# genetics-statistics/GEMMA

Measured on AMD Instinct MI355X. Metric: SNPs/s (-lmm 1 Wald) at n=20k on 1/2/4/8 MI355X; U^T x HBM GB/s vs roofline, higher is better.
Workload: dtype f64 (U^T x as int8-digit MFMA products with exact int32 accumulation; every column of U scaled by its exact maximum and rounded to 6 base-256 digits = 2^-48 of that maximum -- fp64 keeps 2^-53 per entry; value_strict / strict_leg (7g6m: U^T x at or below the fp64 GEMM's own error) and fp64_gemm_path

## Files before the change

gemma_amd/csrc/abi_lmm_multi.inc.h:

```cpp

static int multi_make_weights(hipStream_t s) {
  g_ctx.multi_G = 0;
  const size_t T = g_ctx.multi_T, c = g_ctx.cfg.n_cvt;
  const Ctx::PhenoSlot &p0 = g_ctx.slots[0];
  if (!p0.proto.have_grid || !table_v2_enabled() || p0.grid_geom.nbx != 2) return GEMMA_HIP_OK;
  const int G = std::min(MULTI_GMAX, MULTI_NBA * 16 / p0.grid_geom.nq - (int)c);
  if (G < 2 || T < 2) return GEMMA_HIP_OK;
  const GridGeom gg = p0.grid_geom;
  const size_t r_elems = (size_t)gg.nc * (size_t)(gg.nbx + MULTI_NBA) * 256;
  const size_t groups = (T + G - 1) / G;
  if (g_ctx.multi_R.reserve(groups * r_elems * 8))
    return fail(GEMMA_HIP_ENOMEM, "lmm_multi_setup: weights of the shared table (%zu bytes)", groups * r_elems * 8);
  AssocArgs k = p0.proto;
  k.eval = g_ctx.eval;
  k.UtWt = g_ctx.UtWt.as<double>();
  for (size_t grp = 0; grp < groups; ++grp) {
    MultiWeights mw;
    mw.G = (int)std::min((size_t)G, T - grp * G);
    for (int g = 0; g < MULTI_GMAX; ++g) mw.Uty[g] = g_ctx.slots[std::min(T - 1, grp * G + g)].Uty;
    hipLaunchKernelGGL(grid_weights_multi_kernel, dim3((unsigned)((r_elems + 255) / 256)), dim3(256), 0, s, k, gg, (int)c, mw,
                       g_ctx.multi_R.as<double>() + grp * r_elems);
    HIPCHK(hipGetLastError());
  }
  g_ctx.multi_G = G;
  return GEMMA_HIP_OK;
}

static int multi_setup_slots(size_t T, const double *l_mle_null, const double *logl_mle_H0, const double *UtW_d,
                             const double *UtY_d, hipStream_t s) {
  const size_t n = g_ctx.cfg.n;
  if (g_ctx.multi_Yt.reserve(T * n * 8)) return fail(GEMMA_HIP_ENOMEM, "lmm_multi_setup: U^T Y (%zu bytes)", T * n * 8);
  {
    dim3 grid((unsigned)((T + 31) / 32), (unsigned)((n + 31) / 32));
    hipLaunchKernelGGL(transpose_kernel, grid, dim3(32, 8), 0, s, UtY_d, (long)n, (long)T, (long)T, g_ctx.multi_Yt.as<double>(),
                       (long)n);
    HIPCHK(hipGetLastError());
  }
  g_ctx.slots.clear();
  g_ctx.slots.resize(T);
  g_ctx.multi_T = T;
  for (size_t t = 0; t < T; ++t) {
    Ctx::PhenoSlot &p = g_ctx.slots[t];
    p.proto = t == 0 ? g_ctx.single.proto : g_ctx.slots[0].proto;
    if (p.carry.reserve(4 * 8)) return fail(GEMMA_HIP_ENOMEM, "lmm_multi_setup: carry");
    HIPCHK(hipMemset(p.carry.p, 0, 4 * 8));
    p.carry_flip = 0;
    p.proto.l_mle_null = l_mle_null ? l_mle_null[t] : 0.0;
    p.proto.logl_mle_H0 = logl_mle_H0 ? logl_mle_H0[t] : 0.0;
    p.Uty = g_ctx.multi_Yt.as<double>() + t * n;
    const int rc = t == 0 ? make_utwt(p, UtW_d, s) : make_grid(p, s);
    if (rc == GEMMA_HIP_ENOMEM) {
      const Ctx::PhenoSlot &p0 = g_ctx.slots[0];
      const size_t per = p0.grid_R.cap + p0.grid_F.cap + p0.cheb_R.cap + p0.cheb_F.cap;
      return fail(GEMMA_HIP_ENOMEM, "lmm_multi_setup: the tables of phenotype %zu of %zu do not fit (%zu bytes per phenotype)", t + 1, T,
                  per);
    }
    if (rc) return rc;
  }
  return multi_make_weights(s);
}

static int multi_check(const gemma_lmm_cfg *cfg, size_t T, const double *l_mle_null, const double *logl_mle_H0) {
  if (!cfg) return fail(GEMMA_HIP_EINVAL, "lmm_multi_setup: null cfg");
  if (T == 0 || T > (size_t)GEMMA_LMM_MULTI_MAX)
    return fail(GEMMA_HIP_EINVAL, "lmm_multi_setup: T=%zu phenotypes (1..%d)", T, GEMMA_LMM_MULTI_MAX);
  if (cfg->a_mode != 1 && (!l_mle_null || !logl_mle_H0))
    return fail(GEMMA_HIP_EINVAL, "lmm_multi_setup: a_mode %d needs l_mle_null and logl_mle_H0 of every phenotype", cfg->a_mode);
  return GEMMA_HIP_OK;
}
static int multi_setup(const char *who, SetupSrc src, const gemma_lmm_cfg *cfg, size_t T, const double *l_mle_null,
                       const double *logl_mle_H0, const double *U, const double *eval, const double *UtW, const double *UtY,
                       hipStream_t s) {
  const double *UtW_d, *UtY_d;
  int rc = lmm_bind(who, src, cfg, U, eval, UtW, UtY, T, &UtW_d, &UtY_d);
  if (rc) return rc;
  if ((rc = multi_setup_slots(T, l_mle_null, logl_mle_H0, UtW_d, UtY_d, s))) {
    multi_release();
    return rc;
  }
  if (src != SetupSrc::Device) HIPCHK(hipDeviceSynchronize());
  g_ctx.lmm_active = true;
  return GEMMA_HIP_OK;
}

extern "C" int gemma_hip_lmm_multi_setup_d(const gemma_lmm_cfg *cfg, size_t T, const double *l_mle_null,
                                           const double *logl_mle_H0, const double *U_d, const double *eval_d,
                                           const double *UtW_d, const double *UtY_d, void *stream) {
  NEED_INIT();
  if (!U_d || !eval_d || !UtW_d || !UtY_d) return fail(GEMMA_HIP_EINVAL, "lmm_multi_setup: null pointer");
  if (int rc = multi_check(cfg, T, l_mle_null, logl_mle_H0)) return rc;
  return multi_setup("lmm_multi_setup", SetupSrc::Device, cfg, T, l_mle_null, logl_mle_H0, U_d, eval_d, UtW_d, UtY_d, S(stream));
}

extern "C" int gemma_hip_lmm_multi_setup(const gemma_lmm_cfg *cfg, size_t T, const double *l_mle_null, const double *logl_mle_H0,
                                         const double *U, const double *eval, const double *UtW, const double *UtY) {
  NEED_INIT();
  if (!U || !eval || !UtW || !UtY) return fail(GEMMA_HIP_EINVAL, "lmm_multi_setup: null pointer");
  if (int rc = multi_check(cfg, T, l_mle_null, logl_mle_H0)) return rc;
  return multi_setup("lmm_multi_setup", SetupSrc::Host, cfg, T, l_mle_null, logl_mle_H0, U, eval, UtW, UtY, nullptr);
}

extern "C" int gemma_hip_lmm_multi_setup_kept(const gemma_lmm_cfg *cfg, size_t T, const double *l_mle_null,
                                              const double *logl_mle_H0, const double *UtW, const double *UtY) {
  NEED_INIT();
  if (!g_ctx.kept_n) return fail(GEMMA_HIP_ESTATE, "lmm_multi_setup_kept: no kept U");
  if (!UtW || !UtY) return fail(GEMMA_HIP_EINVAL, "lmm_multi_setup_kept: null pointer");
  if (int rc = multi_check(cfg, T, l_mle_null, logl_mle_H0)) return rc;
  if (cfg->n != g_ctx.kept_n)
    return fail(GEMMA_HIP_EINVAL, "lmm_multi_setup_kept: cfg.n=%zu, kept U is %zu", cfg->n, g_ctx.kept_n);
  return multi_setup("lmm_multi_setup_kept", SetupSrc::Kept, cfg, T, l_mle_null, logl_mle_H0, nullptr, nullptr, UtW, UtY, nullptr);
}

static int launch_table_multi(size_t grp, int Gn, const double *UtX, size_t l, size_t ld, hipStream_t s) {
  const Ctx::PhenoSlot &p0 = g_ctx.slots[0];
  const GridGeom &gg = p0.grid_geom;
  constexpr int NB16M = (2 + MULTI_NBA) * 16;
  const size_t nb16 = (size_t)p0.proto.grid_ld;
  const int ksplit = table_ksplit(gg.nc);
  if (g_ctx.table_P.reserve((size_t)ksplit * l * NB16M * 8) || g_ctx.multi_T_buf.reserve((size_t)Gn * l * nb16 * 8))
    return fail(GEMMA_HIP_ENOMEM, "lmm_multi_batch: shared table partial sums (%zu bytes)", (size_t)ksplit * l * NB16M * 8);
  const size_t r_elems = (size_t)gg.nc * (size_t)(gg.nbx + MULTI_NBA) * 256;
  TableV2 a;
  a.UtX = UtX; a.ld = (long)ld; a.l = (long)l; a.n = (int)g_ctx.cfg.n; a.nc = gg.nc; a.ksplit = ksplit;
  a.Rp = g_ctx.multi_R.as<double>() + grp * r_elems;
  a.P = g_ctx.table_P.as<double>(); a.cap = (long)l;
  a.tg = TableGather();
  const size_t rows_per_block = (size_t)MULTI_RG * 16 * 4;
  const dim3 grid((unsigned)((l + rows_per_block - 1) / rows_per_block), (unsigned)ksplit);
  if (g_ctx.knobs.table_pf) hipLaunchKernelGGL((table_v2_kernel<2, MULTI_NBA, MULTI_RG, false, true>), grid, dim3(256), 0, s, a);
  else hipLaunchKernelGGL((table_v2_kernel<2, MULTI_NBA, MULTI_RG, false, false>), grid, dim3(256), 0, s, a);
  HIPCHK(hipGetLastError());
  TableMulti m;
  m.P = a.P; m.ksplit = ksplit; m.cap = (long)l; m.l = (long)l; m.nb16m = NB16M; m.nb16 = (int)nb16;
  m.y0 = p0.proto.grid_xa0 + (int)g_ctx.cfg.n_cvt * gg.nq; m.nq = gg.nq;
  m.T = g_ctx.multi_T_buf.as<double>(); m.tstride = (long)(l * nb16);
  hipLaunchKernelGGL(table_multi_reduce_kernel, dim3((unsigned)((l * nb16 + 255) / 256), (unsigned)Gn), dim3(256), 0, s, m);
  HIPCHK(hipGetLastError());
  return GEMMA_HIP_OK;
}

extern "C" int gemma_hip_lmm_multi_batch_d(int kind, const void *geno, size_t l, size_t ld, gemma_sumstat *out_d, void *stream) {
  NEED_INIT();
  if (!g_ctx.lmm_active || !g_ctx.multi_T) return fail(GEMMA_HIP_ESTATE, "lmm_multi_batch before lmm_multi_setup");
  if (l == 0) return GEMMA_HIP_OK;
  int rc = block_geom("lmm_multi_batch", kind, g_ctx.cfg.n, true, geno, l, ld, out_d);
  if (rc) return rc;
  hipStream_t s = S(stream);
  double *UtX;
  size_t ldx;
  if ((rc = compute_utx(kind, geno, l, ld, -1, &UtX, &ldx, s))) return rc;
  const size_t T = g_ctx.multi_T;
  bool shared = g_ctx.knobs.multi_table && g_ctx.multi_G >= 2 && table_v2_enabled() &&
                assoc_takes_tables(g_ctx.slots[0].proto, UtX, ldx);
  const size_t G = shared ? (size_t)g_ctx.multi_G : 1;
  const size_t tstride = l * (size_t)g_ctx.slots[0].proto.grid_ld;
  for (size_t t0 = 0; t0 < T; t0 += G) {
    const size_t Gn = std::min(G, T - t0);
    if (shared) {
      ProfScope ps(GEMMA_STAGE_ASSOC, s);
      rc = launch_table_multi(t0 / G, (int)Gn, UtX, l, ldx, s);
      if (rc && rc != GEMMA_HIP_ENOMEM) return rc;
      if (rc) shared = false;
    }
    for (size_t g = 0; g < Gn; ++g) {
      rc = launch_assoc(g_ctx.slots[t0 + g], UtX, l, ldx, out_d + (t0 + g) * l, s,
                        shared ? g_ctx.multi_T_buf.as<double>() + g * tstride : nullptr);
      if (rc) return rc;
    }
  }
  return GEMMA_HIP_OK;
}

extern "C" int gemma_hip_lmm_multi_batch(int kind, const void *geno, size_t l, size_t ld, gemma_sumstat *out) {
  NEED_INIT();
  if (!g_ctx.lmm_active || !g_ctx.multi_T) return fail(GEMMA_HIP_ESTATE, "lmm_multi_batch before lmm_multi_setup");
  if (l == 0) return GEMMA_HIP_OK;
  return host_batch("lmm_multi_batch", kind, geno, l, ld, g_ctx.stage_out, out, g_ctx.multi_T * l * sizeof(gemma_sumstat),
                    [&](const void *in_d, void *out_d) {
                      return gemma_hip_lmm_multi_batch_d(kind, in_d, l, ld, static_cast<gemma_sumstat *>(out_d), nullptr);
                    });
}
```

gemma_amd/csrc/abi_lmm_stage.inc.h:

```cpp

static void multi_release() {
  for (auto &p : g_ctx.slots) p.release();
  g_ctx.slots.clear();
  g_ctx.multi_Yt.release(); g_ctx.multi_R.release(); g_ctx.multi_T_buf.release();
  g_ctx.multi_T = 0;
  g_ctx.multi_G = 0;
}
static void score_release() {
  g_ctx.score_R.release(); g_ctx.score_Pyy.release(); g_ctx.score_Yt.release(); g_ctx.score_lam.release(); g_ctx.score_bad.release();
  g_ctx.score_fthr.release(); g_ctx.score_cells.release(); g_ctx.score_hits.release(); g_ctx.score_cnt.release(); g_ctx.score_best.release();
  g_ctx.score_fthr_p = -1.0;
  g_ctx.score_T = 0;
  g_ctx.refine_Yt.release(); g_ctx.refine_logl.release(); g_ctx.refine_out.release();
  g_ctx.refine_ready = false;
  g_ctx.last_UtX = nullptr;
}
static void lmm_release() {
  g_ctx.own_U.release(); g_ctx.own_eval.release(); g_ctx.own_Uty.release(); g_ctx.own_UtW.release();
  g_ctx.UtWt.release(); g_ctx.idx_map.release(); g_ctx.X.release(); g_ctx.UtX.release();
  g_ctx.stage_in.release(); g_ctx.stage_out.release(); g_ctx.scratch.release();
  g_ctx.single.release();
  g_ctx.grid_T.release();
  g_ctx.table_P.release();
  g_ctx.cheb_T.release(); g_ctx.cheb_slots.release();
  g_ctx.cheb_list.release(); g_ctx.cheb_count.release(); g_ctx.cheb_D.release(); g_ctx.cheb_Ck.release();
  g_ctx.cheb_Gk.release(); g_ctx.cheb_Lk.release(); g_ctx.cheb_iv.release(); g_ctx.cheb_dends.release(); g_ctx.cheb_res.release();
  g_ctx.i8_Bt.release(); g_ctx.i8_q.release(); g_ctx.i8_qinv.release(); g_ctx.i8_cmax.release(); g_ctx.i8_A.release(); g_ctx.i8_C.release();
  raster_release();
  g_ctx.i8_mean.release(); g_ctx.i8_meta.release(); g_ctx.i8_rowsur.release(); g_ctx.i8_colsum.release(); g_ctx.i8_surlist.release();
  g_ctx.i8_ready = g_ctx.i8_colsum_ready = false;
  g_ctx.gxe_env.release(); g_ctx.gxe_UtWt.release(); g_ctx.gxe_Z.release(); g_ctx.gxe_UtZ.release(); g_ctx.gxe_flip.release();
  g_ctx.gxe_ready = false;
  g_ctx.mv_Yt.release(); g_ctx.mv_out.release(); g_ctx.mv_scratch.release();
  g_ctx.mv_ready = g_ctx.mv_gxe = false;
  multi_release();
  score_release();
  g_ctx.U = g_ctx.eval = nullptr;
  g_ctx.U_even_of = nullptr;
  g_ctx.U_even.release();
  g_ctx.lmm_active = false;
}
#define NEED_SINGLE(who)                                                                                                 \
  do {                                                                                                                    \
    if (g_ctx.multi_T)                                                                                                    \
      return fail(GEMMA_HIP_ESTATE, who ": the setup holds %zu phenotypes (gemma_hip_lmm_multi_batch)", g_ctx.multi_T);   \
    if (g_ctx.score_T)                                                                                                    \
      return fail(GEMMA_HIP_ESTATE, who ": the setup is a score panel of %zu phenotypes (gemma_hip_lmm_score_panel_batch)", \
                  g_ctx.score_T);                                                                                         \
  } while (0)

static void fill_lam_grid(AssocArgs &a, double l_min, double l_max, size_t n_region) {
  const double lambda_interval = log(l_max / l_min) / (double)n_region;
  for (size_t i = 0; i <= n_region; ++i) a.lam_grid[i] = l_min * exp(lambda_interval * (double)i);
}
static double lnbeta_half(double df) { return lgamma(df / 2.0) + lgamma(0.5) - lgamma(df / 2.0 + 0.5); }
static void null_derive(const NullOut &h, double trace_G, size_t n, size_t n_cvt, double *out8) {
  out8[0] = h.l_mle; out8[1] = h.logl_mle; out8[2] = h.l_remle; out8[3] = h.logl_remle;
  double arg = -1.0 / h.dev2_remle, d1 = arg;
  if (arg < 0.001) d1 = fabs(arg);
  const double se = (d1 < 0.0) ? NAN : sqrt(d1);
  out8[4] = trace_G * h.l_remle / (trace_G * h.l_remle + 1.0);
  out8[5] = trace_G / ((trace_G * h.l_remle + 1.0) * (trace_G * h.l_remle + 1.0)) * se;
  out8[7] = h.Pyy_remle / (double)(n - n_cvt);
  out8[6] = out8[7] * h.l_remle;
}

static int lmm_common_setup(const gemma_lmm_cfg *cfg) {
  if (!cfg) return fail(GEMMA_HIP_EINVAL, "lmm_setup: null cfg");
  if (cfg->n == 0 || cfg->n_cvt == 0) return fail(GEMMA_HIP_EINVAL, "lmm_setup: n=%zu n_cvt=%zu", cfg->n, cfg->n_cvt);
  if (cfg->n_cvt > (size_t)GEN_CMAX_WIDE)
    return fail(GEMMA_HIP_EINVAL, "lmm_setup: n_cvt=%zu not supported by this build (1..%d)", cfg->n_cvt, GEN_CMAX_WIDE);
  if (!(cfg->a_mode == 1 || cfg->a_mode == 2 || cfg->a_mode == 3 || cfg->a_mode == 4 || cfg->a_mode == 9))
    return fail(GEMMA_HIP_EINVAL, "lmm_setup: a_mode %d", cfg->a_mode);
  if (!(cfg->l_max > cfg->l_min) || cfg->n_region == 0 || cfg->n_region > (size_t)ASSOC_MAX_REGION)
    return fail(GEMMA_HIP_EINVAL, "lmm_setup: l_min/l_max/n_region");
  if (cfg->n <= cfg->n_cvt + 1) return fail(GEMMA_HIP_EINVAL, "lmm_setup: n <= n_cvt + 1");
  if (cfg->n > 0x7fffffffUL) return fail(GEMMA_HIP_EINVAL, "lmm_setup: n too large");
  g_ctx.cfg = *cfg;
  if (g_ctx.multi_T) multi_release();
  if (g_ctx.score_T) score_release();
  {
    size_t mf = 0, mt = 0;
    if (eigh_pool_idle_bytes_x() > 0 && hipMemGetInfo(&mf, &mt) == hipSuccess && eigh_pool_idle_bytes_x() > mt / 4) (void)eigh_release_x();
  }
  g_ctx.knobs.load();
  Ctx::PhenoSlot &p = g_ctx.single;
  AssocArgs &a = p.proto;
  memset(&a, 0, sizeof a);
  a.n = (int)cfg->n;
  a.a_mode = cfg->a_mode;
  a.n_region = (int)cfg->n_region;
  a.plink_nan_rule = cfg->plink_nan_rule;
  a.l_min = cfg->l_min;
  a.l_max = cfg->l_max;
  a.l_mle_null = cfg->l_mle_null;
  a.logl_mle_H0 = cfg->logl_mle_H0;
  a.lnbeta_half_df = lnbeta_half((double)cfg->n - (double)cfg->n_cvt - 1.0);
  fill_lam_grid(a, cfg->l_min, cfg->l_max, cfg->n_region);
  if (p.carry.reserve(4 * 8)) return fail(GEMMA_HIP_ENOMEM, "lmm_setup: carry");
  HIPCHK(hipMemset(p.carry.p, 0, 4 * 8));
  p.carry_flip = 0;
  g_ctx.have_map = false;
  g_ctx.ni_total = 0;
  g_ctx.i8_ready = false;
  g_ctx.i8_colsum_ready = false;
  g_ctx.gxe_ready = false;
  g_ctx.mv_ready = false;
  return GEMMA_HIP_OK;
}

static double *kept_U() { return g_ctx.kept_UE.as<double>(); }
static double *kept_eval() { return g_ctx.kept_UE.as<double>() + g_ctx.kept_n * g_ctx.kept_n; }

enum class SetupSrc { Device, Host, Kept };

static int lmm_bind(const char *who, SetupSrc src, const gemma_lmm_cfg *cfg, const double *U, const double *eval, const double *UtW,
                    const double *UtY, size_t T, const double **UtW_d, const double **UtY_d) {
  const int rc = lmm_common_setup(cfg);
  if (rc) return rc;
  g_ctx.lmm_active = false;
  g_ctx.U_even_of = nullptr;
  if (src == SetupSrc::Device) {
    g_ctx.U = U;
    g_ctx.eval = eval;
    *UtW_d = UtW;
    *UtY_d = UtY;
    return GEMMA_HIP_OK;
  }
  const size_t n = cfg->n, c = cfg->n_cvt;
  const bool kept = src == SetupSrc::Kept;
  if ((!kept && (g_ctx.own_U.reserve(n * n * 8) || g_ctx.own_eval.reserve(n * 8))) || g_ctx.own_Uty.reserve(n * T * 8) ||
      g_ctx.own_UtW.reserve(n * c * 8))
    return fail(GEMMA_HIP_ENOMEM, "%s: cannot allocate U and U^T Y (%zu bytes)", who, (kept ? 0 : n * n * 8) + n * T * 8);
  if (!kept) {
    HIPCHK(hipMemcpy(g_ctx.own_U.p, U, n * n * 8, hipMemcpyHostToDevice));
    HIPCHK(hipMemcpy(g_ctx.own_eval.p, eval, n * 8, hipMemcpyHostToDevice));
  }
  HIPCHK(hipMemcpy(g_ctx.own_Uty.p, UtY, n * T * 8, hipMemcpyHostToDevice));
  HIPCHK(hipMemcpy(g_ctx.own_UtW.p, UtW, n * c * 8, hipMemcpyHostToDevice));
  g_ctx.U = kept ? kept_U() : g_ctx.own_U.as<double>();
  g_ctx.eval = kept ? kept_eval() : g_ctx.own_eval.as<double>();
  *UtW_d = g_ctx.own_UtW.as<double>();
  *UtY_d = g_ctx.own_Uty.as<double>();
  return GEMMA_HIP_OK;
}

static bool grid_blocks(size_t c, int nq, int *nbx, int *nba) {
  *nbx = (nq + 15) / 16;
  *nba = ((int)(c + 1) * nq + 15) / 16;
  return c >= 1 && c <= 4 && nq == 23;
}
static int make_cheb(Ctx::PhenoSlot &p, hipStream_t s) {
  AssocArgs &a = p.proto;
  a.have_cheb = 0;
  a.cheb_T = nullptr; a.cheb_F = nullptr; a.cheb_slots = nullptr; a.cheb_res = nullptr;
  if (!g_ctx.knobs.assoc_cheb) return GEMMA_HIP_OK;
  const size_t n = g_ctx.cfg.n, c = g_ctx.cfg.n_cvt;
  const int nreg = (int)g_ctx.cfg.n_region;
  const double width = log(g_ctx.cfg.l_max / g_ctx.cfg.l_min) / (double)nreg;
  if (c < 1 || c > 4 || width > 2.31 || nreg > 62) return GEMMA_HIP_OK;
  int j0 = 0;
  if (!g_ctx.knobs.cheb_lowlambda)
    while (j0 < nreg && a.lam_grid[j0] < CHEB_MIN_LAMBDA * (1.0 - 1e-9)) ++j0;
  const int nint = nreg - j0;
  p.cheb_qmask = 0;
  if (nint <= 0) return GEMMA_HIP_OK;
  GridGeom gg;
  gg.nq = CHEB_N;
  gg.nbx = (CHEB_N + 15) / 16;
  gg.nba = ((int)(c + 1) * CHEB_N + 15) / 16;
  gg.nc = (int)((n + 15) / 16);
  if (!(gg.nbx == 2 && (gg.nba == 3 || gg.nba == 5 || gg.nba == 6 || gg.nba == 8))) return GEMMA_HIP_OK;
  const size_t nb = (size_t)(gg.nbx + gg.nba);
  const size_t r_elems = (size_t)gg.nc * nb * 256;
  const size_t npairs = (c + 1) * (c + 2) / 2;
  const size_t fld = (npairs + 3) * CHEB_N;
  if (p.cheb_R.reserve((size_t)nint * r_elems * 8) || p.cheb_F.reserve((size_t)nint * fld * 8) ||
      g_ctx.cheb_D.reserve(CHEB_N * CHEB_N * 8) || g_ctx.cheb_Ck.reserve(n * CHEB_N * 8) ||
      g_ctx.cheb_Gk.reserve(2 * n * CHEB_N * 8) || g_ctx.cheb_Lk.reserve(n * CHEB_N * 8) ||
      g_ctx.cheb_iv.reserve(2 * ASSOC_MAX_REGION * 8))
    return fail(GEMMA_HIP_ENOMEM, "lmm_setup: Chebyshev tables (%zu bytes)", (size_t)nint * r_elems * 8);
  std::vector<double> D((size_t)CHEB_N * CHEB_N);
  for (int k = 0; k < CHEB_N; ++k)
    for (int m = 0; m < CHEB_N; ++m)
      D[(size_t)k * CHEB_N + m] = cos(M_PI * k * (m + 0.5) / CHEB_N) * (k == 0 ? 1.0 : 2.0) / CHEB_N;
  HIPCHK(hipMemcpyAsync(g_ctx.cheb_D.p, D.data(), D.size() * 8, hipMemcpyHostToDevice, s));
  HIPCHK(hipStreamSynchronize(s));
  AssocArgs k = a;
  k.eval = g_ctx.eval;
  k.Uty = p.Uty;
  k.UtWt = g_ctx.UtWt.as<double>();
  for (int q = 0; q < nint; ++q) {
    const ChebInterval iv = cheb_interval(a.lam_grid[j0 + q], a.lam_grid[j0 + q + 1], CHEB_MARGIN);
    p.cheb_mid[q] = iv.mid;
    p.cheb_inv_half[q] = 1.0 / iv.half;
    ChebNodes nd;
    for (int m = 0; m < CHEB_N; ++m) nd.lam[m] = exp(cheb_node(iv, m));
    const int qform = a.lam_grid[j0 + q] < CHEB_MIN_LAMBDA * (1.0 - 1e-9) ? 1 : 0;
    if (qform) p.cheb_qmask |= 1ull << q;
    double *G2k = g_ctx.cheb_Gk.as<double>() + n * CHEB_N;
    hipLaunchKernelGGL(cheb_coeff_kernel, dim3((unsigned)((n + 127) / 128)), dim3(128), 0, s, g_ctx.eval, (int)n, nd,
                       g_ctx.cheb_D.as<double>(), qform, g_ctx.cheb_Ck.as<double>(), g_ctx.cheb_Gk.as<double>(),
                       g_ctx.cheb_Lk.as<double>(), G2k);
    HIPCHK(hipGetLastError());
    hipLaunchKernelGGL(cheb_weights_kernel, dim3((unsigned)((r_elems + 255) / 256)), dim3(256), 0, s, k, gg, (int)c,
                       g_ctx.cheb_Ck.as<double>(), p.cheb_R.as<double>() + (size_t)q * r_elems);
    HIPCHK(hipGetLastError());
    hipLaunchKernelGGL(cheb_fixed_kernel, dim3((unsigned)(npairs + 3)), dim3(256), 0, s, k, (int)c,
                       g_ctx.cheb_Ck.as<double>(), g_ctx.cheb_Gk.as<double>(), g_ctx.cheb_Lk.as<double>(), G2k,
                       p.cheb_F.as<double>() + (size_t)q * fld);
    HIPCHK(hipGetLastError());
  }
  {
    std::vector<double> ivs(2 * (size_t)nint);
    for (int q = 0; q < nint; ++q) { ivs[2 * q] = p.cheb_mid[q]; ivs[2 * q + 1] = p.cheb_inv_half[q]; }
    HIPCHK(hipMemcpyAsync(g_ctx.cheb_iv.p, ivs.data(), ivs.size() * 8, hipMemcpyHostToDevice, s));
    HIPCHK(hipStreamSynchronize(s));
  }
  p.cheb_geom = gg;
  a.cheb_iv = g_ctx.cheb_iv.as<double>();
  a.cheb_logdet_off = (int)((npairs + 1) * CHEB_N);
  a.cheb_F = p.cheb_F.as<double>();
  a.cheb_ld = (int)(nb * 16);
  a.cheb_fld = (int)fld;
  a.cheb_xa0 = gg.nbx * 16;
  a.cheb_j0 = j0;
  a.cheb_nint = nint;
  a.cheb_qmask = p.cheb_qmask;
  a.cheb_final = g_ctx.knobs.assoc_final_series;
  a.have_cheb = 1;
  return GEMMA_HIP_OK;
}

static int make_grid(Ctx::PhenoSlot &p, hipStream_t s) {
  AssocArgs &a = p.proto;
  a.have_grid = 0;
  a.grid_T = nullptr;
  a.grid_F = nullptr;
  if (!g_ctx.knobs.assoc_grid) return GEMMA_HIP_OK;
  const size_t n = g_ctx.cfg.n, c = g_ctx.cfg.n_cvt;
  GridGeom gg;
  gg.nq = 1 + 2 * ((int)g_ctx.cfg.n_region + 1);
  if (!grid_blocks(c, gg.nq, &gg.nbx, &gg.nba)) return GEMMA_HIP_OK;
  gg.nc = (int)((n + 15) / 16);
  const size_t nb = (size_t)(gg.nbx + gg.nba);
  const size_t r_elems = (size_t)gg.nc * nb * 256;
  if (p.grid_R.reserve(r_elems * 8) || p.grid_F.reserve((size_t)gg.nq * GRID_FIX_LD * 8))
    return fail(GEMMA_HIP_ENOMEM, "lmm_setup: fixed-lambda table");
  AssocArgs k = a;
  k.eval = g_ctx.eval;
  k.Uty = p.Uty;
  k.UtWt = g_ctx.UtWt.as<double>();
  hipLaunchKernelGGL(grid_weights_kernel, dim3((unsigned)((r_elems + 255) / 256)), dim3(256), 0, s, k, gg, (int)c,
                     p.grid_R.as<double>());
  HIPCHK(hipGetLastError());
  hipLaunchKernelGGL(grid_fixed_kernel, dim3((unsigned)gg.nq), dim3(256), 0, s, k, (int)c, p.grid_F.as<double>());
  HIPCHK(hipGetLastError());
  p.grid_geom = gg;
  a.grid_F = p.grid_F.as<double>();
  a.grid_ld = (int)(nb * 16);
  a.grid_nq = gg.nq;
  a.grid_xa0 = gg.nbx * 16;
  a.have_grid = 1;
  return make_cheb(p, s);
}

static bool table_v2_enabled() { return g_ctx.knobs.table_v2 != 0; }
static int table_ksplit(int nc) { return std::max(1, std::min(16, nc / 32)); }
template <int NBX, int NBA, int RG>
static int launch_table_v2_t(const GridGeom &gg, const double *UtX, size_t l, size_t ld, const double *R, double *T,
                             const TableGather *tg, int nint, hipStream_t s) {
  constexpr int NB16 = (NBX + NBA) * 16;
  const size_t rows_per_block = (size_t)RG * 16 * 4;
  const size_t bx = (l + rows_per_block - 1) / rows_per_block;
  const int ksplit = table_ksplit(gg.nc);
  const size_t planes = tg ? (size_t)nint : 1;
  if (g_ctx.table_P.reserve(planes * (size_t)ksplit * l * NB16 * 8))
    return fail(GEMMA_HIP_ENOMEM, "lmm_assoc: table partial sums (%zu bytes)", planes * (size_t)ksplit * l * NB16 * 8);
  TableV2 a;
  a.UtX = UtX; a.ld = (long)ld; a.l = (long)l; a.n = (int)g_ctx.cfg.n; a.nc = gg.nc; a.ksplit = ksplit; a.Rp = R;
  a.P = g_ctx.table_P.as<double>(); a.cap = (long)l;
  if (tg) a.tg = *tg; else a.tg = TableGather();
  const long total = (long)l * NB16;
  const bool pf = g_ctx.knobs.table_pf != 0;
  if (tg) {
    if (pf) hipLaunchKernelGGL((table_v2_kernel<NBX, NBA, RG, true, true>), dim3((unsigned)bx, (unsigned)ksplit, (unsigned)nint), dim3(256), 0, s, a);
    else hipLaunchKernelGGL((table_v2_kernel<NBX, NBA, RG, true, false>), dim3((unsigned)bx, (unsigned)ksplit, (unsigned)nint), dim3(256), 0, s, a);
    HIPCHK(hipGetLastError());
    hipLaunchKernelGGL(table_reduce_kernel<true>, dim3((unsigned)((total + 255) / 256), (unsigned)nint), dim3(256), 0, s,
                       a.P, ksplit, a.cap, NB16, (long)l, tg->count, T);
  } else {
    if (pf) hipLaunchKernelGGL((table_v2_kernel<NBX, NBA, RG, false, true>), dim3((unsigned)bx, (unsigned)ksplit), dim3(256), 0, s, a);
    else hipLaunchKernelGGL((table_v2_kernel<NBX, NBA, RG, false, false>), dim3((unsigned)bx, (unsigned)ksplit), dim3(256), 0, s, a);
    HIPCHK(hipGetLastError());
    hipLaunchKernelGGL(table_reduce_kernel<false>, dim3((unsigned)((total + 255) / 256)), dim3(256), 0, s, a.P, ksplit,
                       a.cap, NB16, (long)l, (const int *)nullptr, T);
  }
  HIPCHK(hipGetLastError());
  return GEMMA_HIP_OK;
}
static int launch_table_v2(const GridGeom &gg, const double *UtX, size_t l, size_t ld, const double *R, double *T,
                           const TableGather *tg, int nint, hipStream_t s) {
  switch (gg.nba) {
  case 3: return launch_table_v2_t<2, 3, 4>(gg, UtX, l, ld, R, T, tg, nint, s);
  case 5: return launch_table_v2_t<2, 5, 2>(gg, UtX, l, ld, R, T, tg, nint, s);
  case 6: return launch_table_v2_t<2, 6, 2>(gg, UtX, l, ld, R, T, tg, nint, s);
  case 8: return launch_table_v2_t<2, 8, 2>(gg, UtX, l, ld, R, T, tg, nint, s);
  default: return fail(GEMMA_HIP_ERUNTIME, "lmm_assoc: no table kernel for %d column blocks", gg.nba);
  }
}

static int launch_grid_table(Ctx::PhenoSlot &p, const double *UtX, size_t l, size_t ld, hipStream_t s) {
  const GridGeom &gg = p.grid_geom;
  const size_t nb = (size_t)(gg.nbx + gg.nba);
  if (g_ctx.grid_T.reserve(l * nb * 16 * 8)) return fail(GEMMA_HIP_ENOMEM, "lmm_assoc: fixed-lambda table");
  const unsigned grid = (unsigned)((l + 15) / 16);
  const double *R = p.grid_R.as<double>();
  double *T = g_ctx.grid_T.as<double>();
  const int n = (int)g_ctx.cfg.n;
  if (table_v2_enabled()) return launch_table_v2(gg, UtX, l, ld, R, T, nullptr, 0, s);
  switch (gg.nba) {
  case 3: hipLaunchKernelGGL((grid_table_kernel<2, 3, false>), dim3(grid), dim3(256), 0, s, UtX, (long)ld, (long)l, n, gg.nc, R, T, TableGather()); break;
  case 5: hipLaunchKernelGGL((grid_table_kernel<2, 5, false>), dim3(grid), dim3(256), 0, s, UtX, (long)ld, (long)l, n, gg.nc, R, T, TableGather()); break;
  case 6: hipLaunchKernelGGL((grid_table_kernel<2, 6, false>), dim3(grid), dim3(256), 0, s, UtX, (long)ld, (long)l, n, gg.nc, R, T, TableGather()); break;
  case 8: hipLaunchKernelGGL((grid_table_kernel<2, 8, false>), dim3(grid), dim3(256), 0, s, UtX, (long)ld, (long)l, n, gg.nc, R, T, TableGather()); break;
  default: return fail(GEMMA_HIP_ERUNTIME, "lmm_assoc: no fixed-lambda table kernel for %d column blocks", gg.nba);
  }
  HIPCHK(hipGetLastError());
  return GEMMA_HIP_OK;
}

static int launch_cheb_tables(Ctx::PhenoSlot &p, AssocArgs &a, const double *UtX, size_t l, size_t ld, hipStream_t s) {
  const GridGeom &gg = p.cheb_geom;
  const size_t nb = (size_t)(gg.nbx + gg.nba), nint = (size_t)a.cheb_nint;
  if (g_ctx.cheb_T.reserve(nint * l * nb * 16 * 8) || g_ctx.cheb_slots.reserve(l * nint * sizeof(int)) ||
      g_ctx.cheb_list.reserve(nint * l * sizeof(int)) || g_ctx.cheb_count.reserve(ASSOC_MAX_REGION * sizeof(int)) ||
      g_ctx.cheb_dends.reserve(2 * nint * l * sizeof(double2)) || g_ctx.cheb_res.reserve(2 * nint * l * sizeof(ChebResult)))
    return fail(GEMMA_HIP_ENOMEM, "lmm_assoc: Chebyshev tables of the batch (%zu bytes)", nint * l * nb * 16 * 8);
  HIPCHK(hipMemsetAsync(g_ctx.cheb_count.p, 0, ASSOC_MAX_REGION * sizeof(int), s));
  a.cheb_T = g_ctx.cheb_T.as<double>();
  a.cheb_cap = (long)l;
  ChebScanArgs sc;
  sc.count = g_ctx.cheb_count.as<int>();
  sc.list = g_ctx.cheb_list.as<int>();
  sc.slots = g_ctx.cheb_slots.as<int>();
  sc.dends = g_ctx.cheb_dends.as<double2>();
  sc.cap = (long)l;
  const unsigned sgrid = (unsigned)((l + 3) / 4);
  const size_t c = g_ctx.cfg.n_cvt;
  switch (c) {
  case 1: hipLaunchKernelGGL(cheb_scan_kernel<1>, dim3(sgrid), dim3(256), 0, s, a, sc); break;
  case 2: hipLaunchKernelGGL(cheb_scan_kernel<2>, dim3(sgrid), dim3(256), 0, s, a, sc); break;
  case 3: hipLaunchKernelGGL(cheb_scan_kernel<3>, dim3(sgrid), dim3(256), 0, s, a, sc); break;
  default: hipLaunchKernelGGL(cheb_scan_kernel<4>, dim3(sgrid), dim3(256), 0, s, a, sc); break;
  }
  HIPCHK(hipGetLastError());
  TableGather tg;
  tg.list = sc.list;
  tg.count = sc.count;
  tg.cap = (long)l;
  tg.rp_stride = (long)gg.nc * (long)nb * 256;
  const dim3 grid((unsigned)((l + 15) / 16), (unsigned)nint);
  const double *R = p.cheb_R.as<double>();
  double *T = g_ctx.cheb_T.as<double>();
  const int n = (int)g_ctx.cfg.n;
  if (table_v2_enabled()) {
    int rc = launch_table_v2(gg, UtX, l, ld, R, T, &tg, (int)nint, s);
    if (rc) return rc;
  } else
  switch (gg.nba) {
  case 3: hipLaunchKernelGGL((grid_table_kernel<2, 3, true>), grid, dim3(256), 0, s, UtX, (long)ld, (long)l, n, gg.nc, R, T, tg); break;
  case 5: hipLaunchKernelGGL((grid_table_kernel<2, 5, true>), grid, dim3(256), 0, s, UtX, (long)ld, (long)l, n, gg.nc, R, T, tg); break;
  case 6: hipLaunchKernelGGL((grid_table_kernel<2, 6, true>), grid, dim3(256), 0, s, UtX, (long)ld, (long)l, n, gg.nc, R, T, tg); break;
  case 8: hipLaunchKernelGGL((grid_table_kernel<2, 8, true>), grid, dim3(256), 0, s, UtX, (long)ld, (long)l, n, gg.nc, R, T, tg); break;
  default: return fail(GEMMA_HIP_ERUNTIME, "lmm_assoc: no table kernel for %d column blocks", gg.nba);
  }
  HIPCHK(hipGetLastError());
  ChebSearchArgs sa;
  sa.count = sc.count;
  sa.list = sc.list;
  sa.qmask = p.cheb_qmask;
  sa.dends = sc.dends;
  sa.res = g_ctx.cheb_res.as<ChebResult>();
  memcpy(sa.mid, p.cheb_mid, sizeof sa.mid);
  memcpy(sa.inv_half, p.cheb_inv_half, sizeof sa.inv_half);
  const dim3 qgrid((unsigned)((l + 63) / 64), (unsigned)nint, 2);
  switch (c) {
  case 1: hipLaunchKernelGGL(cheb_search_kernel<1>, qgrid, dim3(64), 0, s, a, sa); break;
  case 2: hipLaunchKernelGGL(cheb_search_kernel<2>, qgrid, dim3(64), 0, s, a, sa); break;
  case 3: hipLaunchKernelGGL(cheb_search_kernel<3>, qgrid, dim3(64), 0, s, a, sa); break;
  default: hipLaunchKernelGGL(cheb_search_kernel<4>, qgrid, dim3(64), 0, s, a, sa); break;
  }
  HIPCHK(hipGetLastError());
  a.cheb_slots = sc.slots;
  a.cheb_res = sa.res;
  return GEMMA_HIP_OK;
}

static int make_utwt(Ctx::PhenoSlot &p, const double *UtW_d, hipStream_t s) {
  const size_t n = g_ctx.cfg.n, c = g_ctx.cfg.n_cvt;
  if (g_ctx.UtWt.reserve(c * n * 8)) return fail(GEMMA_HIP_ENOMEM, "lmm_setup: UtWt");
  dim3 grid((unsigned)((c + 31) / 32), (unsigned)((n + 31) / 32));
  hipLaunchKernelGGL(transpose_kernel, grid, dim3(32, 8), 0, s, UtW_d, (long)n, (long)c, (long)c,
                     g_ctx.UtWt.as<double>(), (long)n);
  HIPCHK(hipGetLastError());
  if (g_ctx.scratch.reserve(16)) return fail(GEMMA_HIP_ENOMEM, "lmm_setup: scratch");
  hipLaunchKernelGGL(logdet_ends_kernel, dim3(1), dim3(64), 0, s, g_ctx.eval, (int)n, g_ctx.cfg.l_min, g_ctx.cfg.l_max,
                     g_ctx.scratch.as<double>());
  HIPCHK(hipGetLastError());
  double ends[2];
  HIPCHK(hipMemcpyAsync(ends, g_ctx.scratch.p, 16, hipMemcpyDeviceToHost, s));
  HIPCHK(hipStreamSynchronize(s));
  p.proto.logdet_lmin = ends[0];
  p.proto.logdet_lmax = ends[1];
  p.proto.have_logdet_ends = 1;
  return make_grid(p, s);
}

static int single_setup(const char *who, SetupSrc src, const gemma_lmm_cfg *cfg, const double *U, const double *eval,
                        const double *UtW, const double *Uty, hipStream_t s) {
  const double *UtW_d, *Uty_d;
  int rc = lmm_bind(who, src, cfg, U, eval, UtW, Uty, 1, &UtW_d, &Uty_d);
  if (rc) return rc;
  g_ctx.single.Uty = Uty_d;
  if ((rc = make_utwt(g_ctx.single, UtW_d, s))) return rc;
  if (src != SetupSrc::Device) HIPCHK(hipDeviceSynchronize());
  g_ctx.lmm_active = true;
  return GEMMA_HIP_OK;
}

extern "C" int gemma_hip_lmm_setup_d(const gemma_lmm_cfg *cfg, const double *U_d, const double *eval_d,
                                     const double *UtW_d, const double *Uty_d, void *stream) {
  NEED_INIT();
  if (!U_d || !eval_d || !UtW_d || !Uty_d) return fail(GEMMA_HIP_EINVAL, "lmm_setup: null pointer");
  return single_setup("lmm_setup", SetupSrc::Device, cfg, U_d, eval_d, UtW_d, Uty_d, S(stream));
}

extern "C" int gemma_hip_lmm_setup(const gemma_lmm_cfg *cfg, const double *U, const double *eval,
                                   const double *UtW, const double *Uty) {
  NEED_INIT();
  if (!U || !eval || !UtW || !Uty) return fail(GEMMA_HIP_EINVAL, "lmm_setup: null pointer");
  return single_setup("lmm_setup", SetupSrc::Host, cfg, U, eval, UtW, Uty, nullptr);
}

extern "C" int gemma_hip_lmm_set_indicator(const int *indicator_idv, size_t ni_total) {
  NEED_INIT();
  if (!g_ctx.lmm_active && !g_ctx.lm_active) return fail(GEMMA_HIP_ESTATE, "lmm_set_indicator before lmm_setup / lm_setup");
  if (!indicator_idv || ni_total == 0) {
    g_ctx.have_map = false;
    g_ctx.ni_total = 0;
    return GEMMA_HIP_OK;
  }
  std::vector<int> map;
  map.reserve(g_ctx.cfg.n);
  for (size_t i = 0; i < ni_total; ++i)
    if (indicator_idv[i] != 0) map.push_back((int)i);
  if (map.size() != g_ctx.cfg.n)
    return fail(GEMMA_HIP_EINVAL, "lmm_set_indicator: %zu analysed individuals, cfg.n = %zu", map.size(),
                g_ctx.cfg.n);
  if (map.size() == ni_total) {
    g_ctx.have_map = false;
    g_ctx.ni_total = 0;
    return GEMMA_HIP_OK;
  }
  if (g_ctx.idx_map.reserve(map.size() * sizeof(int))) return fail(GEMMA_HIP_ENOMEM, "idx_map");
  HIPCHK(hipMemcpy(g_ctx.idx_map.p, map.data(), map.size() * sizeof(int), hipMemcpyHostToDevice));
  g_ctx.have_map = true;
  g_ctx.ni_total = ni_total;
  return GEMMA_HIP_OK;
}

static bool assoc_takes_tables(const AssocArgs &a, const double *UtX, size_t ld) {
  const size_t sel = g_ctx.knobs.force_generic ? 99 : g_ctx.cfg.n_cvt;
  return a.have_grid && sel <= 4 && (ld & 1) == 0 && (reinterpret_cast<uintptr_t>(UtX) & 15) == 0 &&
         a.a_mode != 3;
}
static int launch_assoc(Ctx::PhenoSlot &p, const double *UtX, size_t l, size_t ld, gemma_sumstat *out_d, hipStream_t s,
                        const double *shared_T = nullptr) {
  AssocArgs a = p.proto;
  a.UtX = UtX;
  a.ld = (long)ld;
  a.l = (long)l;
  a.eval = g_ctx.eval;
  a.Uty = p.Uty;
  a.UtWt = g_ctx.UtWt.as<double>();
  a.out = reinterpret_cast<SumStat *>(out_d);
  const unsigned grid = (unsigned)((l + 3) / 4);
  {
    ProfScope ps(GEMMA_STAGE_ASSOC, s);
    const size_t sel = g_ctx.knobs.force_generic ? 99 : g_ctx.cfg.n_cvt;
    a.grid_T = nullptr;
    if (assoc_takes_tables(a, UtX, ld)) {
      int rc = shared_T ? GEMMA_HIP_OK : launch_grid_table(p, UtX, l, ld, s);
      if (rc && rc != GEMMA_HIP_ENOMEM) return rc;
      a.grid_T = rc ? nullptr : (shared_T ? shared_T : g_ctx.grid_T.as<double>());
      a.cheb_T = nullptr;
      a.cheb_slots = nullptr;
      a.cheb_res = nullptr;
      if (!rc && a.have_cheb) {
        rc = launch_cheb_tables(p, a, UtX, l, ld, s);
        if (rc && rc != GEMMA_HIP_ENOMEM) return rc;
        if (rc) { a.cheb_T = nullptr; a.cheb_slots = nullptr; a.cheb_res = nullptr; }
      }
    }
    switch (sel) {
    case 1: {
      const int var = g_ctx.knobs.assoc_variant;
      if (var == 43) hipLaunchKernelGGL((lmm_assoc1_variant_kernel<4, 3>), dim3(grid), dim3(256), 0, s, a);
      else if (var == 83) hipLaunchKernelGGL((lmm_assoc1_variant_kernel<8, 3>), dim3(grid), dim3(256), 0, s, a);
      else if (var == 24) hipLaunchKernelGGL((lmm_assoc1_variant_kernel<2, 4>), dim3(grid), dim3(256), 0, s, a);
      else if (var == 23) hipLaunchKernelGGL(lmm_assoc_kernel<1>, dim3(grid), dim3(256), 0, s, a);
      else if (var == 42) hipLaunchKernelGGL((lmm_assoc1_variant_kernel<4, 2>), dim3(grid), dim3(256), 0, s, a);
      else hipLaunchKernelGGL((lmm_assoc1_variant_kernel<4, 4>), dim3(grid), dim3(256), 0, s, a);
      break;
    }
    case 2: hipLaunchKernelGGL(lmm_assoc_kernel<2>, dim3(grid), dim3(256), 0, s, a); break;
    case 3: hipLaunchKernelGGL(lmm_assoc_kernel<3>, dim3(grid), dim3(256), 0, s, a); break;
    case 4: hipLaunchKernelGGL(lmm_assoc_kernel<4>, dim3(grid), dim3(256), 0, s, a); break;
    default:
      if (g_ctx.cfg.n_cvt > (size_t)GEN_CMAX) {
        int rcw = wide_attr(lmm_assoc_wide_kernel);
        if (rcw) return rcw;
        hipLaunchKernelGGL(lmm_assoc_wide_kernel, dim3((unsigned)l), dim3(64), wide_lds_bytes(g_ctx.cfg.n_cvt), s, a,
                           (int)g_ctx.cfg.n_cvt);
      } else {
        hipLaunchKernelGGL(lmm_assoc_generic_kernel, dim3(grid), dim3(256), 0, s, a, (int)g_ctx.cfg.n_cvt);
      }
      break;
    }
    HIPCHK(hipGetLastError());
    if (g_ctx.cfg.plink_nan_rule && g_ctx.cfg.a_mode == 1) {
      double *cin = p.carry.as<double>() + 2 * p.carry_flip;
      double *cout = p.carry.as<double>() + 2 * (1 - p.carry_flip);
      hipLaunchKernelGGL(plink_carry_kernel, dim3((unsigned)((l + 255) / 256)), dim3(256), 0, s,
                         reinterpret_cast<SumStatRaw *>(out_d), (long)l, cin, cout);
      HIPCHK(hipGetLastError());
      p.carry_flip = 1 - p.carry_flip;
    }
  }
  return GEMMA_HIP_OK;
}

extern "C" int gemma_hip_lmm_assoc_d(const double *UtX_d, size_t l, size_t ld_utx, gemma_sumstat *out_d,
                                     void *stream) {
  NEED_INIT();
  if (!g_ctx.lmm_active) return fail(GEMMA_HIP_ESTATE, "lmm_assoc before lmm_setup");
  NEED_SINGLE("lmm_assoc");
  if (l == 0) return GEMMA_HIP_OK;
  if (!UtX_d || !out_d || ld_utx < g_ctx.cfg.n) return fail(GEMMA_HIP_EINVAL, "lmm_assoc: bad UtX/ld");
  {
    int rcf = xp_flush_fwd(S(stream));
    if (rcf) return rcf;
  }
  return launch_assoc(g_ctx.single, UtX_d, l, ld_utx, out_d, S(stream));
}

static int utx_i8_mode() { return g_ctx.knobs.i8.utx_i8; }

static void note_utx_kernel(int variant, int digits, int fuse, int raster) {
  static const char *const names[GEMMA_UTX_KERNEL_COUNT] = {
      "dgemm_mfma_glds_kernel", "i8gemm_packed_kernel_t<true>", "i8gemm_sparse_kernel", "i8gemm_sparse2_kernel",
      "i8gemm_sparse2_r16_kernel", "i8gemm_packed_kernel_t<false, true>", "i8gemm_dense16_kernel_t<true>"};
  gemma_utx_kernel_info &k = g_ctx.last_utx_kernel;
  k.variant = variant;
  k.rows = (variant == GEMMA_UTX_KERNEL_RECORDS_R16 || variant == GEMMA_UTX_KERNEL_DOSAGE_I8_R16) ? 16
                                                                                                   : (variant == GEMMA_UTX_KERNEL_DGEMM_F64 ? 0 : 32);
  k.digits = digits; k.fuse = fuse; k.raster = raster;
  k.launches += 1;
  snprintf(k.name, sizeof k.name, "%s", names[variant]);
}

static size_t round_up(size_t v, size_t m) { return (v + m - 1) / m * m; }

static int i8_digits_for(size_t n) {
  if (g_ctx.knobs.i8_digits) return g_ctx.knobs.i8_digits;
  return n >= 16384 ? 6 : 7;
}

static int i8_prepare_u(hipStream_t s) {
  if (g_ctx.i8_ready) return GEMMA_HIP_OK;
  const size_t n = g_ctx.cfg.n;
  const size_t ldk = round_up(n, I8_BK), npad = round_up(n, I8_BN);
  g_ctx.i8_digits = i8_digits_for(n);
  if (g_ctx.i8_Bt.reserve((size_t)I8_DIGITS * npad * ldk) || g_ctx.i8_q.reserve(n * 8) || g_ctx.i8_qinv.reserve(n * 8) ||
      g_ctx.i8_cmax.reserve(n * 8))
    return fail(GEMMA_HIP_ENOMEM, "lmm_batch: int8 digits of U (%zu bytes)", (size_t)I8_DIGITS * npad * ldk);
  HIPCHK(hipMemsetAsync(g_ctx.i8_Bt.p, 0, (size_t)I8_DIGITS * npad * ldk, s));
  HIPCHK(hipMemsetAsync(g_ctx.i8_cmax.p, 0, n * 8, s));
  hipLaunchKernelGGL(u_colmax_kernel, dim3((unsigned)((n + 255) / 256), (unsigned)((n + 1023) / 1024)), dim3(256), 0, s,
                     g_ctx.U, (long)n, (long)n, g_ctx.i8_cmax.as<unsigned long long>());
  HIPCHK(hipGetLastError());
  hipLaunchKernelGGL(u_scale_kernel, dim3((unsigned)((n + 255) / 256)), dim3(256), 0, s,
                     g_ctx.i8_cmax.as<unsigned long long>(), (long)n, g_ctx.i8_digits, g_ctx.knobs.i8_scale_max,
                     g_ctx.i8_q.as<double>(), g_ctx.i8_qinv.as<double>());
  HIPCHK(hipGetLastError());
  hipLaunchKernelGGL(u_digits_kernel, dim3((unsigned)((n + 31) / 32), (unsigned)((n + 31) / 32)), dim3(256), 0, s,
                     g_ctx.U, (long)n, (long)n, g_ctx.i8_q.as<double>(), g_ctx.i8_Bt.as<int8_t>(), (long)ldk,
                     (long)(npad * ldk), g_ctx.i8_digits);
  HIPCHK(hipGetLastError());
  g_ctx.i8_ldk = ldk;
  g_ctx.i8_npad = npad;
  g_ctx.i8_ready = true;
  return GEMMA_HIP_OK;
}
```

gemma_amd/csrc/gemma_hip.hip:

```cpp
#include <hip/hip_runtime.h>

#include <cmath>
#include <cstdarg>
#include <cstdio>
#include <cstdlib>
#include <cstring>
#include <string>
#include <vector>

#include "../../include/gemma_hip.h"
#include "tu_common.h"
#include "dgemm.h"
#include "eigh_tu.h"
#include "vc_tu.h"
#include "prdt_tu.h"
#include "mqs_tu.h"
#include "cor_tu.h"
#include "ingest.h"
#include "lm_assoc.h"
#include "lmm_assoc.h"
#include "lmm_grid.h"
#include "lmm_score_panel.h"
#include "lmm_null_panel.h"
#include "lmm_pair.h"
#include "i8gemm.h"
#include "i8gemm_sparse.h"
#include "i8gemm_sparse2.h"
#include "i8gemm_sparse2_r16.h"
#include "plink_records.h"
#include "i8gemm_dense16.h"
#include "qc.h"
#include "mvlmm.hip.h"
#include "mvlmm_pair.h"
#include "comm.hip.h"
#include "kin_i8.h"
#include "i8_plan.h"

using namespace gemma_hip;

namespace {

struct StageProf {
  std::vector<std::pair<hipEvent_t, hipEvent_t>> ev;
  double acc_ms = 0.0;
  long launches = 0;
};

struct Knobs {
  I8Switches i8;
  int i8_digits = 0;
  int i8_scale_max = 1;
  int dosage_i8 = 1;
  int dosage_rows = 16;
  int table_v2 = 1;
  int table_pf = 0;
  int multi_table = 1;
  int force_generic = 0;
  int assoc_variant = 44;
  int mvlmm_rt = 0;
  int pipe_cus = 64;
  int kin_i8 = 1, kin_upper = 1, kin_lists = 1, kin_lists_oom = 0;
  long long kin_list_cap = 0;
  int assoc_grid = 1;
  int assoc_cheb = 1;
  int cheb_lowlambda = 1;
  int assoc_final_series = 1;
  static int geti(const char *name, int dflt) {
    const char *e = getenv(name);
    return (e && *e) ? atoi(e) : dflt;
  }
  static int on_unless_0(const char *name) {
    const char *e = getenv(name);
    return (e && e[0] == '0') ? 0 : 1;
  }
  static int off_unless_1(const char *name) {
    const char *e = getenv(name);
    return (e && e[0] == '1') ? 1 : 0;
  }
  void load() {
    i8.utx_i8 = geti("GEMMA_HIP_UTX_I8", 1);
    const int dg = geti("GEMMA_HIP_I8_DIGITS", 0);
    i8_digits = (dg == 6 || dg == 7) ? dg : 0;
    const char *es = getenv("GEMMA_HIP_I8_SPARSE");
    i8.sparse = (es && es[0] >= '0' && es[0] <= '2') ? es[0] - '0' : 2;
    i8.fuse = on_unless_0("GEMMA_HIP_I8_FUSE");
    i8.gm = geti("GEMMA_HIP_I8_GM", 0);
    i8.raster = geti("GEMMA_HIP_I8_RASTER", S2_DEFAULT_RASTER);
    i8.rows = geti("GEMMA_HIP_I8_ROWS", 16) == 32 ? 32 : 16;
    const char *esc = getenv("GEMMA_HIP_I8_SCALE");
    i8_scale_max = (esc && strcmp(esc, "pow2") == 0) ? 0 : 1;
    const char *efm = getenv("GEMMA_HIP_I8_FORM");
    i8.mdrop = (efm && strcmp(efm, "7g6m") == 0) ? 1 : 0;
    if (i8.mdrop) i8_digits = 7;
    i8.complete = on_unless_0("GEMMA_HIP_I8_COMPLETE");
    i8.epilogue = on_unless_0("GEMMA_HIP_I8_EPILOGUE");
    i8.epi_depth = geti("GEMMA_HIP_I8_EPI_DEPTH", 4) <= 1 ? 1 : 4;
    i8.direct = on_unless_0("GEMMA_HIP_I8_DIRECT");
    dosage_i8 = on_unless_0("GEMMA_HIP_UTX_DOSAGE_I8");
    dosage_rows = geti("GEMMA_HIP_DOSAGE_ROWS", 16) == 32 ? 32 : 16;
    i8.overlap = off_unless_1("GEMMA_HIP_OVERLAP");
    i8.chunks = geti("GEMMA_HIP_OVERLAP_CHUNKS", 4);
    table_v2 = on_unless_0("GEMMA_HIP_TABLE_V2");
    table_pf = off_unless_1("GEMMA_HIP_TABLE_PF");
    multi_table = on_unless_0("GEMMA_HIP_MULTI_TABLE");
    force_generic = off_unless_1("GEMMA_HIP_FORCE_GENERIC");
    assoc_variant = geti("GEMMA_HIP_ASSOC_VARIANT", 44);
    mvlmm_rt = off_unless_1("GEMMA_HIP_MVLMM_RT");
    pipe_cus = geti("GEMMA_HIP_PIPE_CUS", 64);
    kin_i8 = on_unless_0("GEMMA_HIP_KIN_I8");
    kin_upper = on_unless_0("GEMMA_HIP_KIN_UPPER");
    kin_lists = on_unless_0("GEMMA_HIP_KIN_LISTS");
    kin_lists_oom = off_unless_1("GEMMA_HIP_KIN_LISTS_OOM");
    const char *kc = getenv("GEMMA_HIP_KIN_LIST_CAP");
    kin_list_cap = (kc && *kc) ? atoll(kc) : 0;
    assoc_grid = on_unless_0("GEMMA_HIP_ASSOC_GRID");
    assoc_cheb = on_unless_0("GEMMA_HIP_ASSOC_CHEB");
    cheb_lowlambda = on_unless_0("GEMMA_HIP_CHEB_LOWLAMBDA");
    assoc_final_series = on_unless_0("GEMMA_HIP_ASSOC_FINAL_SERIES");
  }
};

struct Ctx {
  bool inited = false;
  Knobs knobs;
  int device = -1;
  int verbose = 0;
  std::string last_error;
  hipDeviceProp_t prop;
  bool profiling = false;
  StageProf prof[GEMMA_STAGE_COUNT];

  bool kin_active = false;
  size_t kin_n = 0;
  int kin_mode = 1;
  size_t kin_ns = 0;
  DevBuf kin_K, kin_X, kin_stage;
  hipStream_t kin_copy = nullptr;
  hipEvent_t kin_copied = nullptr, kin_ingested = nullptr;
  bool kin_ingested_valid = false, kin_host_call = false;
  DevBuf qc_G, qc_M, qc_W, qc_O;
  bool kin_i8 = false, kin_i8_used = false;
  DevBuf i8_meta, i8_rowsur;
  DevBuf U_even;
  const double *U_even_of = nullptr;
  DevBuf kin_GtG, kin_S, kin_a, kin_At, kin_Gt;
  DevBuf kin_A2, kin_cnt, kin_off, kin_listS, kin_listJ, kin_sub, kin_cj, kin_flag;
  DevBuf kin_tmap;
  hipStream_t ov_stream = nullptr;
  hipEvent_t ov_ready[16] = {}, ov_done = nullptr;
  struct XPipe {
    hipStream_t P = nullptr, Q = nullptr;
    hipEvent_t in_ready = nullptr, prod_done[2] = {}, post_done[2] = {};
    hipEvent_t ingest_done = nullptr;
    bool ingest_valid = false;
    bool post_valid[2] = {false, false};
    unsigned long long count = 0;
    bool pending = false;
    int cus = -1;
    DevBuf shadow_A, shadow_C, shadow_mean, shadow_rowsur;
  } xp;
  int kin_tmap_tm = 0, kin_tmap_tn = 0, kin_tmap_count = 0;

  bool lmm_active = false;
  gemma_lmm_cfg cfg;
  const double *U = nullptr, *eval = nullptr;
  DevBuf own_U, own_eval, own_Uty, own_UtW, UtWt, idx_map;
  size_t ni_total = 0;
  bool have_map = false;
  DevBuf X, UtX, stage_in, stage_out;
  DevBuf grid_T;
  DevBuf cheb_T, cheb_slots, cheb_list, cheb_count, cheb_D, cheb_Ck, cheb_Gk, cheb_Lk, cheb_iv, cheb_dends, cheb_res;
  DevBuf table_P;
  DevBuf gxe_env, gxe_UtWt, gxe_Z, gxe_UtZ, gxe_flip;
  bool gxe_ready = false;
  double gxe_lnbeta = 0.0;
  DevBuf mv_Yt, mv_out;
  DevBuf mv_scratch;
  bool mv_ready = false, mv_gxe = false;
  size_t mv_d = 0;
  MvArgs mv_proto;
  struct MvLast {
    int form = 0, d = 0, rows = 0;
  } mv_last[2];
  DevBuf i8_Bt, i8_q, i8_qinv, i8_cmax, i8_A, i8_C, i8_mean;
  struct RasterSlot {
    DevBuf dev;
    std::vector<int2> host;
    int tm = 0, tn = 0, rb = 0, xcds = 8;
    unsigned long long used = 0;
  } i8_raster[6];
  unsigned long long i8_raster_clock = 0;
  DevBuf i8_surlist;
  DevBuf i8_colsum;
  bool i8_colsum_ready = false;
  int last_utx_path = 0;
  gemma_utx_kernel_info last_utx_kernel = {};
  int i8_last_epi = -1;
  long i8_rowsur_n = 0;
  long i8_flag_at = -1;
  bool i8_ready = false;
  size_t i8_ldk = 0, i8_npad = 0;
  int i8_digits = I8_DIGITS;
  struct PhenoSlot {
    AssocArgs proto;
    const double *Uty = nullptr;
    DevBuf grid_R, grid_F, cheb_R, cheb_F;
    DevBuf carry;
    GridGeom grid_geom, cheb_geom;
    double cheb_mid[ASSOC_MAX_REGION], cheb_inv_half[ASSOC_MAX_REGION];
    unsigned long long cheb_qmask = 0;
    int carry_flip = 0;
    void release() {
      grid_R.release(); grid_F.release(); cheb_R.release(); cheb_F.release(); carry.release();
      Uty = nullptr;
    }
  };
  PhenoSlot single;
  std::vector<PhenoSlot> slots;
  size_t multi_T = 0;
  DevBuf multi_Yt;
  DevBuf multi_R, multi_T_buf;
  int multi_G = 0;
  size_t score_T = 0;
  ScoreGeom score_geom;
  DevBuf score_R, score_Pyy, score_Yt, score_lam, score_bad;
  DevBuf score_fthr, score_cells, score_hits, score_cnt, score_best;
  double score_fthr_p = -1.0;
  hipStream_t score_fthr_s = nullptr;
  bool refine_ready = false;
  DevBuf refine_Yt, refine_logl;
  DevBuf refine_out;
  AssocArgs refine_proto;
  const double *last_UtX = nullptr;
  size_t last_l = 0, last_ldx = 0;

  bool lm_active = false;
  LmArgs lm_proto;
  DevBuf lm_Wt, lm_y, lm_small;

  DevBuf scratch;

  struct PipeSlot {
    void *pin_in = nullptr, *pin_out = nullptr;
    size_t pin_in_cap = 0, pin_out_cap = 0;
    DevBuf dev_in, dev_out;
    hipEvent_t h2d = nullptr, done = nullptr;
    size_t l = 0;
    bool busy = false;
  } pipe[2];
  hipStream_t pipe_copy = nullptr, pipe_comp = nullptr;
  int pipe_head = 0, pipe_count = 0;

  DevBuf kept_K, kept_UE;
  size_t kept_K_n = 0, kept_n = 0;
  double kept_trace = 0.0;
  Comm comm;
} g_ctx;

int fail(int code, const char *fmt, ...) {
  char buf[512];
  va_list ap;
  va_start(ap, fmt);
  vsnprintf(buf, sizeof buf, fmt, ap);
  va_end(ap);
  g_ctx.last_error = buf;
  if (g_ctx.verbose) fprintf(stderr, "gemma_hip: %s\n", buf);
  return code;
}

int ret(int rc, const std::string &msg) { return rc ? fail(rc, "%s", msg.c_str()) : GEMMA_HIP_OK; }

#define HIPCHK(expr)                                                                        \
  do {                                                                                      \
    hipError_t e_ = (expr);                                                                 \
    if (e_ != hipSuccess)                                                                   \
      return fail(GEMMA_HIP_ERUNTIME, "%s failed: %s (%s:%d)", #expr, hipGetErrorString(e_), \
                  __FILE__, __LINE__);                                                      \
  } while (0)

#define NEED_INIT()                                                                              \
  do {                                                                                           \
    if (!g_ctx.inited) {                                                                         \
      int rc_ = gemma_hip_init(-1, 0);                                                           \
      if (rc_ != GEMMA_HIP_OK) return rc_;                                                       \
    }                                                                                            \
  } while (0)

struct ProfScope {
  int stage;
  hipStream_t s;
  hipEvent_t a = nullptr, b = nullptr;
  ProfScope(int st, hipStream_t stream) : stage(st), s(stream) {
    if (g_ctx.profiling) {
      if (hipEventCreate(&a) == hipSuccess && hipEventCreate(&b) == hipSuccess)
        (void)hipEventRecord(a, s);
      else
        a = b = nullptr;
    }
  }
  ~ProfScope() {
    if (a && b) {
      (void)hipEventRecord(b, s);
      g_ctx.prof[stage].ev.emplace_back(a, b);
    }
  }
};

int prof_collect(int stage) {
  StageProf &p = g_ctx.prof[stage];
  for (auto &pr : p.ev) {
    (void)hipEventSynchronize(pr.second);
    float ms = 0.f;
    if (hipEventElapsedTime(&ms, pr.first, pr.second) == hipSuccess) {
      p.acc_ms += ms;
      p.launches += 1;
    }
    (void)hipEventDestroy(pr.first);
    (void)hipEventDestroy(pr.second);
  }
  p.ev.clear();
  return GEMMA_HIP_OK;
}

inline hipStream_t S(void *s) { return reinterpret_cast<hipStream_t>(s); }

}

static void pipe_release();
static void xp_release();
static int xp_flush_fwd(hipStream_t s);
static void raster_release() {
  for (auto &r : g_ctx.i8_raster) {
    r.dev.release();
    r.host.clear();
    r.tm = r.tn = r.rb = 0;
    r.used = 0;
  }
}
static void qc_release() { g_ctx.qc_G.release(); g_ctx.qc_M.release(); g_ctx.qc_W.release(); g_ctx.qc_O.release(); }
static void kin_i8_release();
static void kin_release();
static void lmm_release();
static void lm_release();

extern "C" int gemma_hip_abi_version(void) { return GEMMA_HIP_ABI_VERSION; }

extern "C" const char *gemma_hip_strerror(int code) {
  switch (code) {
  case GEMMA_HIP_OK: return "ok";
  case GEMMA_HIP_EINVAL: return "invalid argument (range error)";
  case GEMMA_HIP_ENODEV: return "no usable gfx950 device";
  case GEMMA_HIP_ENOMEM: return "device memory allocation failed";
  case GEMMA_HIP_ERUNTIME: return "HIP runtime error";
  case GEMMA_HIP_ESTATE: return "call sequence violated";
  case GEMMA_HIP_ENOCONV: return "eigensolver did not converge";
  case GEMMA_HIP_ENOTPD: return "matrix not positive definite";
  default: return "unknown error";
  }
}

extern "C" const char *gemma_hip_last_error(void) { return g_ctx.last_error.c_str(); }

extern "C" int gemma_hip_init(int device, int verbose) {
  g_ctx.verbose = verbose;
  int ndev = 0;
  if (hipGetDeviceCount(&ndev) != hipSuccess || ndev <= 0) {
    (void)hipGetLastError();
    return fail(GEMMA_HIP_ENODEV, "no HIP device visible (this library has no CPU fallback)");
  }
  if (device >= 0) {
    if (device >= ndev) return fail(GEMMA_HIP_ENODEV, "device %d out of range (%d visible)", device, ndev);
    HIPCHK(hipSetDevice(device));
  }
  int cur = 0;
  HIPCHK(hipGetDevice(&cur));
  HIPCHK(hipGetDeviceProperties(&g_ctx.prop, cur));
  if (strncmp(g_ctx.prop.gcnArchName, "gfx950", 6) != 0)
    return fail(GEMMA_HIP_ENODEV, "device %d is %s; this build targets gfx950 only", cur,
                g_ctx.prop.gcnArchName);
  g_ctx.device = cur;
  g_ctx.inited = true;
  g_ctx.knobs.load();
  gemm_aux_init();
  if (verbose)
    fprintf(stderr, "gemma_hip: device %d %s (%s), %d CUs, %.1f GB\n", cur, g_ctx.prop.name,
            g_ctx.prop.gcnArchName, g_ctx.prop.multiProcessorCount,
            (double)g_ctx.prop.totalGlobalMem / 1e9);
  return GEMMA_HIP_OK;
}

extern "C" void gemma_hip_shutdown(void) {
  if (!g_ctx.inited) return;
  (void)hipDeviceSynchronize();
  for (int s = 0; s < GEMMA_STAGE_COUNT; ++s) prof_collect(s);
  kin_release();
  qc_release();
  lmm_release();
  lm_release();
  pipe_release();
  xp_release();
  if (g_ctx.ov_stream) {
    (void)hipStreamDestroy(g_ctx.ov_stream);
    for (auto &e : g_ctx.ov_ready)
      if (e) (void)hipEventDestroy(e);
    if (g_ctx.ov_done) (void)hipEventDestroy(g_ctx.ov_done);
    g_ctx.ov_stream = nullptr;
    for (auto &e : g_ctx.ov_ready) e = nullptr;
    g_ctx.ov_done = nullptr;
  }
  if (g_ctx.kin_copy) {
    (void)hipStreamDestroy(g_ctx.kin_copy);
    if (g_ctx.kin_copied) (void)hipEventDestroy(g_ctx.kin_copied);
    if (g_ctx.kin_ingested) (void)hipEventDestroy(g_ctx.kin_ingested);
    g_ctx.kin_copy = nullptr;
    g_ctx.kin_copied = g_ctx.kin_ingested = nullptr;
    g_ctx.kin_ingested_valid = false;
  }
  g_ctx.kept_K.release(); g_ctx.kept_UE.release();
  g_ctx.kept_K_n = g_ctx.kept_n = 0;
  g_ctx.comm.finalize();
  gemm_aux_destroy();
  eigh_tu_shutdown();
  vc_tu_shutdown();
  prdt_tu_shutdown();
  mqs_tu_shutdown();
  cor_tu_shutdown();
  g_ctx.inited = false;
}

extern "C" int gemma_hip_device_info(char *name, size_t len, int *n_cu, size_t *hbm_bytes) {
  NEED_INIT();
  if (name && len) {
    snprintf(name, len, "%s (%s)", g_ctx.prop.name, g_ctx.prop.gcnArchName);
  }
  if (n_cu) *n_cu = g_ctx.prop.multiProcessorCount;
  if (hbm_bytes) *hbm_bytes = g_ctx.prop.totalGlobalMem;
  return GEMMA_HIP_OK;
}

extern "C" int gemma_hip_profile_enable(int on) {
  g_ctx.profiling = (on != 0);
  return GEMMA_HIP_OK;
}

extern "C" int gemma_hip_profile_read(int stage, double *total_ms, long *launches, int reset) {
  NEED_INIT();
  if (stage < 0 || stage >= GEMMA_STAGE_COUNT) return fail(GEMMA_HIP_EINVAL, "bad stage %d", stage);
  prof_collect(stage);
  if (total_ms) *total_ms = g_ctx.prof[stage].acc_ms;
  if (launches) *launches = g_ctx.prof[stage].launches;
  if (reset) {
    g_ctx.prof[stage].acc_ms = 0.0;
    g_ctx.prof[stage].launches = 0;
  }
  return GEMMA_HIP_OK;
}

static int check_gemm(char ta, char tb, size_t M, size_t N, size_t K, size_t lda, size_t ldb,
                      size_t ldc) {
  const bool tA = (ta == 'T' || ta == 't'), tB = (tb == 'T' || tb == 't');
  if (!tA && ta != 'N' && ta != 'n') return fail(GEMMA_HIP_EINVAL, "dgemm: bad TransA '%c'", ta);
  if (!tB && tb != 'N' && tb != 'n') return fail(GEMMA_HIP_EINVAL, "dgemm: bad TransB '%c'", tb);
  const size_t a_cols = tA ? M : K, b_cols = tB ? K : N;
  if (lda < a_cols || ldb < b_cols || ldc < N)
    return fail(GEMMA_HIP_EINVAL, "Range error in dgemm (lda=%zu ldb=%zu ldc=%zu for M=%zu N=%zu K=%zu)",
                lda, ldb, ldc, M, N, K);
  return GEMMA_HIP_OK;
}

extern "C" int gemma_hip_dgemm_d(char ta, char tb, size_t M, size_t N, size_t K, double alpha,
                                 const double *A, size_t lda, const double *B, size_t ldb,
                                 double beta, double *C, size_t ldc, void *stream) {
  NEED_INIT();
  int rc = check_gemm(ta, tb, M, N, K, lda, ldb, ldc);
  if (rc) return rc;
  if (M == 0 || N == 0) return GEMMA_HIP_OK;
  ProfScope ps(GEMMA_STAGE_UTX_GEMM, S(stream));
  HIPCHK(launch_dgemm(ta, tb, (long)M, (long)N, (long)K, alpha, A, (long)lda, B, (long)ldb, beta, C,
                      (long)ldc, false, false, S(stream)));
  return GEMMA_HIP_OK;
}

extern "C" int gemma_hip_dgemm(char ta, char tb, size_t M, size_t N, size_t K, double alpha,
                               const double *A, size_t lda, const double *B, size_t ldb,
                               double beta, double *C, size_t ldc) {
  NEED_INIT();
  int rc = check_gemm(ta, tb, M, N, K, lda, ldb, ldc);
  if (rc) return rc;
  if (M == 0 || N == 0) return GEMMA_HIP_OK;
  const bool tA = (ta == 'T' || ta == 't'), tB = (tb == 'T' || tb == 't');
  const size_t a_rows = tA ? K : M, b_rows = tB ? N : K;
  const size_t a_bytes = a_rows * lda * 8, b_bytes = b_rows * ldb * 8, c_bytes = M * ldc * 8;
  ScopedBuf dA, dB, dC;
  if (dA.reserve(a_bytes ? a_bytes : 8) || dB.reserve(b_bytes ? b_bytes : 8) || dC.reserve(c_bytes))
    return fail(GEMMA_HIP_ENOMEM, "dgemm: cannot allocate %zu bytes", a_bytes + b_bytes + c_bytes);
  auto h2d = [&](void *d, const double *h, size_t rows, size_t cols, size_t ld) -> hipError_t {
    if (rows == 0 || cols == 0) return hipSuccess;
    return hipMemcpy2D(d, ld * 8, h, ld * 8, cols * 8, rows, hipMemcpyHostToDevice);
  };
  HIPCHK(h2d(dA.p, A, a_rows, tA ? M : K, lda));
  HIPCHK(h2d(dB.p, B, b_rows, tB ? K : N, ldb));
  if (beta != 0.0) HIPCHK(h2d(dC.p, C, M, N, ldc));
  HIPCHK(launch_dgemm(ta, tb, (long)M, (long)N, (long)K, alpha, dA.as<double>(), (long)lda, dB.as<double>(), (long)ldb, beta,
                      dC.as<double>(), (long)ldc, false, false, 0));
  HIPCHK(hipMemcpy2D(C, ldc * 8, dC.p, ldc * 8, N * 8, M, hipMemcpyDeviceToHost));
  return GEMMA_HIP_OK;
}

#include "abi_host_block.inc.h"
#include "abi_kinship.inc.h"
#include "abi_eigen_qc.inc.h"
#include "abi_lmm_stage.inc.h"
#include "abi_utx.inc.h"
#include "abi_lmm_batch.inc.h"
#include "abi_gxe_lm.inc.h"
#include "abi_mvlmm.inc.h"
#include "abi_kept_comm.inc.h"
#include "abi_lmm_multi.inc.h"
#include "abi_lmm_score_panel.inc.h"
#include "abi_lmm_score_refine.inc.h"
#include "abi_lmm_null_panel.inc.h"
#include "abi_mvlmm_pairs.inc.h"
#include "abi_vc.inc.h"
#include "abi_prdt.inc.h"
#include "abi_mqs.inc.h"
#include "abi_cor.inc.h"
```

gemma_amd/csrc/lmm_grid.h:

```cpp
#pragma once
#include <hip/hip_runtime.h>
#include "dgemm.h"
#include "lmm_assoc.h"

namespace gemma_hip {

constexpr int GRID_FIX_LD = 16;

struct GridGeom {
  int nq;
  int nbx;
  int nba;
  int nc;
};

__global__ void grid_weights_kernel(AssocArgs g, GridGeom gg, int c, double *__restrict__ Rp);

__global__ __launch_bounds__(256) void grid_fixed_kernel(AssocArgs g, int c, double *__restrict__ F);

struct TableGather {
  const int *list;
  const int *count;
  long cap;
  long rp_stride;
};

template <int NBX, int NBA, bool GATHER>
__global__ __launch_bounds__(256) void grid_table_kernel(const double *__restrict__ UtX, long ld, long l, int n,
                                                        int nc, const double *__restrict__ Rp,
                                                        double *__restrict__ T, TableGather tg);

struct TableV2 {
  const double *UtX;
  long ld;
  long l;
  int n, nc;
  int ksplit;
  const double *Rp;
  double *P;
  long cap;
  TableGather tg;
};

template <int NBX, int NBA, int RG, bool GATHER, bool PF>
__global__ __launch_bounds__(256, PF ? 1 : 2) void table_v2_kernel(TableV2 a);

template <bool GATHER>
__global__ __launch_bounds__(256) void table_reduce_kernel(const double *__restrict__ P, int ksplit, long cap, int nb16,
                                                          long l, const int *__restrict__ count, double *__restrict__ T);

constexpr int MULTI_NBA = 8, MULTI_RG = 2, MULTI_GMAX = 4;
struct MultiWeights {
  const double *Uty[MULTI_GMAX];
  int G;
};

__global__ void grid_weights_multi_kernel(AssocArgs g, GridGeom gg, int c, MultiWeights mw, double *__restrict__ Rp);
struct TableMulti {
  const double *P;
  int ksplit;
  long cap, l;
  int nb16m;
  int nb16;
  int y0, nq;
  double *T;
  long tstride;
};

__global__ __launch_bounds__(256) void table_multi_reduce_kernel(TableMulti m);

constexpr double CHEB_MARGIN = 0.15;
constexpr double CHEB_MIN_LAMBDA = 1e-3;

struct ChebNodes {
  double lam[CHEB_N];
};

__global__ void cheb_coeff_kernel(const double *__restrict__ eval, int n, ChebNodes nd, const double *__restrict__ Dfit,
                                  int qform, double *__restrict__ Ck, double *__restrict__ Gk, double *__restrict__ Lk,
                                  double *__restrict__ G2k);

__global__ void cheb_weights_kernel(AssocArgs g, GridGeom gg, int c, const double *__restrict__ Ck,
                                    double *__restrict__ Rp);

__global__ __launch_bounds__(256) void cheb_fixed_kernel(AssocArgs g, int c, const double *__restrict__ Ck,
                                                        const double *__restrict__ Gk, const double *__restrict__ Lk,
                                                        const double *__restrict__ G2k, double *__restrict__ F);

struct ChebScanArgs {
  int *count;
  int *list;
  int *slots;
  double2 *dends;
  long cap;
};

template <int C>
__global__ __launch_bounds__(256) void cheb_scan_kernel(AssocArgs g, ChebScanArgs sc);

struct ChebSearchArgs {
  const int *count;
  const int *list;
  unsigned long long qmask;
  const double2 *dends;
  ChebResult *res;
  double mid[ASSOC_MAX_REGION], inv_half[ASSOC_MAX_REGION];
};

template <int C>
__global__ __launch_bounds__(64) void cheb_search_kernel(AssocArgs g, ChebSearchArgs sa);

#define LMM_GRID_INSTANCES(T) \
  T void grid_table_kernel<2, 3, false>(const double *, long, long, int, int, const double *, double *, TableGather); \
  T void grid_table_kernel<2, 3, true>(const double *, long, long, int, int, const double *, double *, TableGather); \
  T void grid_table_kernel<2, 5, false>(const double *, long, long, int, int, const double *, double *, TableGather); \
  T void grid_table_kernel<2, 5, true>(const double *, long, long, int, int, const double *, double *, TableGather); \
  T void grid_table_kernel<2, 6, false>(const double *, long, long, int, int, const double *, double *, TableGather); \
  T void grid_table_kernel<2, 6, true>(const double *, long, long, int, int, const double *, double *, TableGather); \
  T void grid_table_kernel<2, 8, false>(const double *, long, long, int, int, const double *, double *, TableGather); \
  T void grid_table_kernel<2, 8, true>(const double *, long, long, int, int, const double *, double *, TableGather); \
  T void table_v2_kernel<2, 3, 4, false, false>(TableV2); \
  T void table_v2_kernel<2, 3, 4, false, true>(TableV2); \
  T void table_v2_kernel<2, 3, 4, true, false>(TableV2); \
  T void table_v2_kernel<2, 3, 4, true, true>(TableV2); \
  T void table_v2_kernel<2, 5, 2, false, false>(TableV2); \
  T void table_v2_kernel<2, 5, 2, false, true>(TableV2); \
  T void table_v2_kernel<2, 5, 2, true, false>(TableV2); \
  T void table_v2_kernel<2, 5, 2, true, true>(TableV2); \
  T void table_v2_kernel<2, 6, 2, false, false>(TableV2); \
  T void table_v2_kernel<2, 6, 2, false, true>(TableV2); \
  T void table_v2_kernel<2, 6, 2, true, false>(TableV2); \
  T void table_v2_kernel<2, 6, 2, true, true>(TableV2); \
  T void table_v2_kernel<2, 8, 2, false, false>(TableV2); \
  T void table_v2_kernel<2, 8, 2, false, true>(TableV2); \
  T void table_v2_kernel<2, 8, 2, true, false>(TableV2); \
  T void table_v2_kernel<2, 8, 2, true, true>(TableV2); \
  T void table_reduce_kernel<false>(const double *, int, long, int, long, const int *, double *); \
  T void table_reduce_kernel<true>(const double *, int, long, int, long, const int *, double *); \
  T void cheb_scan_kernel<1>(AssocArgs, ChebScanArgs); \
  T void cheb_scan_kernel<2>(AssocArgs, ChebScanArgs); \
  T void cheb_scan_kernel<3>(AssocArgs, ChebScanArgs); \
  T void cheb_scan_kernel<4>(AssocArgs, ChebScanArgs); \
  T void cheb_search_kernel<1>(AssocArgs, ChebSearchArgs); \
  T void cheb_search_kernel<2>(AssocArgs, ChebSearchArgs); \
  T void cheb_search_kernel<3>(AssocArgs, ChebSearchArgs); \
  T void cheb_search_kernel<4>(AssocArgs, ChebSearchArgs);
#ifndef GEMMA_HIP_KERNEL_BODIES
LMM_GRID_INSTANCES(extern template __global__)
#endif

}
```

gemma_amd/csrc/lmm_grid.hip.h:

```cpp
#pragma once
#include <hip/hip_runtime.h>
#include "dgemm.h"
#include "lmm_assoc.hip.h"
#define GEMMA_HIP_KERNEL_BODIES
#include "lmm_grid.h"

namespace gemma_hip {

__device__ __forceinline__ double grid_weight(const double *__restrict__ eval, const double *lam_grid, int q, long k) {
  if (q == 0) return 1.0;
  const int gi = (q - 1) >> 1;
  const double h = recip(eval[k] * lam_grid[gi] + 1.0);
  return ((q - 1) & 1) ? h * h : h;
}

__global__ void grid_weights_kernel(AssocArgs g, GridGeom gg, int c, double *__restrict__ Rp) {
  const long total = (long)gg.nc * (gg.nbx + gg.nba) * 256;
  const long e = (long)blockIdx.x * blockDim.x + threadIdx.x;
  if (e >= total) return;
  const int j = (int)(e & 3), col = (int)((e >> 2) & 15), kq = (int)((e >> 6) & 3);
  const long r = e >> 8;
  const int nb = gg.nbx + gg.nba;
  const int cb = (int)(r % nb);
  const long chunk = r / nb;
  const long k = chunk * 16 + 4 * kq + j;
  double v = 0.0;
  if (k < g.n) {
    if (cb < gg.nbx) {
      const int q = cb * 16 + col;
      if (q < gg.nq) v = grid_weight(g.eval, g.lam_grid, q, k);
    } else {
      const int idx = (cb - gg.nbx) * 16 + col;
      const int a = idx / gg.nq, q = idx - a * gg.nq;
      if (a <= c) {
        const double u = (a < c) ? g.UtWt[(long)a * g.n + k] : g.Uty[k];
        v = u * grid_weight(g.eval, g.lam_grid, q, k);
      }
    }
  }
  Rp[e] = v;
}

__global__ __launch_bounds__(256) void grid_fixed_kernel(AssocArgs g, int c, double *__restrict__ F) {
  const int q = blockIdx.x;
  const int nv = c + 1;
  double s[GRID_FIX_LD];
#pragma unroll
  for (int p = 0; p < GRID_FIX_LD; ++p) s[p] = 0.0;
  for (long i = threadIdx.x; i < g.n; i += 256) {
    const double w = grid_weight(g.eval, g.lam_grid, q, i);
    s[15] += w;
    int p = 0;
    for (int a = 0; a < nv; ++a) {
      const double ua = (a < c) ? g.UtWt[(long)a * g.n + i] : g.Uty[i];
      for (int b = a; b < nv; ++b) {
        const double ub = (b < c) ? g.UtWt[(long)b * g.n + i] : g.Uty[i];
        if (p < 15) s[p] += ua * ub * w;
        ++p;
      }
    }
  }
  __shared__ double red[4][GRID_FIX_LD];
  const int lane = threadIdx.x & 63, wave = threadIdx.x >> 6;
#pragma unroll
  for (int p = 0; p < GRID_FIX_LD; ++p) {
    const double v = wave_sum(s[p]);
    if (lane == 0) red[wave][p] = v;
  }
  __syncthreads();
  if (threadIdx.x < GRID_FIX_LD)
    F[(long)q * GRID_FIX_LD + threadIdx.x] =
        ((red[0][threadIdx.x] + red[1][threadIdx.x]) + red[2][threadIdx.x]) + red[3][threadIdx.x];
}
template <int NBX, int NBA, bool GATHER>
__global__ __launch_bounds__(256) void grid_table_kernel(const double *__restrict__ UtX, long ld, long l, int n,
                                                        int nc, const double *__restrict__ Rp,
                                                        double *__restrict__ T, TableGather tg) {
  constexpr int NB = NBX + NBA;
  __shared__ double red[3][NB][256];
  const int t = threadIdx.x, lane = t & 63;
  const int wave = __builtin_amdgcn_readfirstlane(t >> 6);
  const int i = lane & 15, kq = lane >> 4;
  const long s0 = (long)blockIdx.x * 16;
  long row = s0 + i;
  if (GATHER) {
    const int kint = blockIdx.y;
    l = tg.count[kint];
    if (s0 >= l) return;
    if (row >= l) row = l - 1;
    row = tg.list[(long)kint * tg.cap + row];
    Rp += (long)kint * tg.rp_stride;
    T += (long)kint * tg.cap * (NB * 16);
  } else {
    if (row >= l) row = l - 1;
  }
  const double *xr = UtX + row * ld + 4 * kq;
  const int c0 = (int)((long)nc * wave / 4), c1 = (int)((long)nc * (wave + 1) / 4);
  f64x4 acc[NB];
#pragma unroll
  for (int b = 0; b < NB; ++b) acc[b] = f64x4{0.0, 0.0, 0.0, 0.0};
  const double *rp = Rp + ((long)c0 * NB * 64 + lane) * 4;
  for (int ch = c0; ch < c1; ++ch) {
    const long k = (long)ch * 16 + 4 * kq;
    double xv[4];
    if (k + 3 < n) {
      const f64x2 lo = *reinterpret_cast<const f64x2 *>(xr + (long)ch * 16);
      const f64x2 hi = *reinterpret_cast<const f64x2 *>(xr + (long)ch * 16 + 2);
      xv[0] = lo.x; xv[1] = lo.y; xv[2] = hi.x; xv[3] = hi.y;
    } else {
#pragma unroll
      for (int j = 0; j < 4; ++j) xv[j] = (k + j < n) ? xr[(long)ch * 16 + j] : 0.0;
    }
    double rb[NB][4];
#pragma unroll
    for (int b = 0; b < NB; ++b) {
      const f64x2 lo = *reinterpret_cast<const f64x2 *>(rp + (long)b * 256);
      const f64x2 hi = *reinterpret_cast<const f64x2 *>(rp + (long)b * 256 + 2);
      rb[b][0] = lo.x; rb[b][1] = lo.y; rb[b][2] = hi.x; rb[b][3] = hi.y;
    }
    rp += (long)NB * 256;
#pragma unroll
    for (int j = 0; j < 4; ++j) {
      const double xs = xv[j] * xv[j];
#pragma unroll
      for (int b = 0; b < NB; ++b)
        acc[b] = __builtin_amdgcn_mfma_f64_16x16x4f64(b < NBX ? xs : xv[j], rb[b][j], acc[b], 0, 0, 0);
    }
  }
  if (wave > 0) {
#pragma unroll
    for (int b = 0; b < NB; ++b)
#pragma unroll
      for (int r = 0; r < 4; ++r) red[wave - 1][b][r * 64 + lane] = acc[b][r];
  }
  __syncthreads();
  if (wave == 0) {
#pragma unroll
    for (int b = 0; b < NB; ++b)
#pragma unroll
      for (int r = 0; r < 4; ++r) {
        const double v = ((acc[b][r] + red[0][b][r * 64 + lane]) + red[1][b][r * 64 + lane]) + red[2][b][r * 64 + lane];
        const long srow = s0 + kq + 4 * r;
        if (srow < l) {
          if (GATHER)
            T[(long)(b * 16 + i) * tg.cap + srow] = v;
          else
            T[srow * (NB * 16) + b * 16 + i] = v;
        }
      }
  }
}
template <int NBX, int NBA, int RG, bool GATHER, bool PF>
__global__ __launch_bounds__(256, PF ? 1 : 2) void table_v2_kernel(TableV2 a) {
  constexpr int NB = NBX + NBA;
  const int lane = threadIdx.x & 63;
  const int wave = __builtin_amdgcn_readfirstlane(threadIdx.x >> 6);
  const int i = lane & 15, kq = lane >> 4;
  const int ks = blockIdx.y;
  const int kint = GATHER ? blockIdx.z : 0;
  long l = a.l;
  const double *Rp = a.Rp;
  if (GATHER) {
    l = a.tg.count[kint];
    Rp += (long)kint * a.tg.rp_stride;
  }
  const long s0 = ((long)blockIdx.x * 4 + wave) * (RG * 16);
  if (s0 >= l) return;
  const double *xr[RG];
#pragma unroll
  for (int g = 0; g < RG; ++g) {
    long row = s0 + g * 16 + i;
    if (row >= l) row = l - 1;
    if (GATHER) row = a.tg.list[(long)kint * a.tg.cap + row];
    xr[g] = a.UtX + row * a.ld + 4 * kq;
  }
  const int c0 = (int)((long)a.nc * ks / a.ksplit), c1 = (int)((long)a.nc * (ks + 1) / a.ksplit);
  f64x4 acc[RG][NB];
#pragma unroll
  for (int g = 0; g < RG; ++g)
#pragma unroll
    for (int b = 0; b < NB; ++b) acc[g][b] = f64x4{0.0, 0.0, 0.0, 0.0};
  const double *rp0 = Rp + (long)lane * 4;
  const int n = a.n;
  const int nfull = n / 16;
  const int cfull = c1 < nfull ? c1 : nfull;
#define TV2_LOAD(RB, XV, CH)                                                                                      \
  do {                                                                                                            \
    const double *rp_ = rp0 + (long)(CH) * NB * 256;                                                              \
    _Pragma("unroll") for (int b = 0; b < NB; ++b) {                                                              \
      const f64x2 lo = *reinterpret_cast<const f64x2 *>(rp_ + (long)b * 256);                                     \
      const f64x2 hi = *reinterpret_cast<const f64x2 *>(rp_ + (long)b * 256 + 2);                                 \
      RB[b][0] = lo.x; RB[b][1] = lo.y; RB[b][2] = hi.x; RB[b][3] = hi.y;                                         \
    }                                                                                                             \
    _Pragma("unroll") for (int g = 0; g < RG; ++g) {                                                              \
      const f64x2 lo = *reinterpret_cast<const f64x2 *>(xr[g] + (long)(CH) * 16);                                 \
      const f64x2 hi = *reinterpret_cast<const f64x2 *>(xr[g] + (long)(CH) * 16 + 2);                             \
      XV[g][0] = lo.x; XV[g][1] = lo.y; XV[g][2] = hi.x; XV[g][3] = hi.y;                                         \
    }                                                                                                             \
  } while (0)
#define TV2_MFMA(RB, XV)                                                                                          \
  do {                                                                                                            \
    _Pragma("unroll") for (int j = 0; j < 4; ++j) {                                                               \
      _Pragma("unroll") for (int g = 0; g < RG; ++g) {                                                            \
        const double xs = XV[g][j] * XV[g][j];                                                                    \
        _Pragma("unroll") for (int b = 0; b < NB; ++b)                                                            \
          acc[g][b] = __builtin_amdgcn_mfma_f64_16x16x4f64(b < NBX ? xs : XV[g][j], RB[b][j], acc[g][b], 0, 0, 0); \
      }                                                                                                           \
    }                                                                                                             \
  } while (0)
  double rbA[NB][4], xvA[RG][4];
  if (PF) {
    double rbB[NB][4], xvB[RG][4];
    if (c0 < cfull) TV2_LOAD(rbA, xvA, c0);
    int ch = c0;
    for (; ch + 1 < cfull; ch += 2) {
      TV2_LOAD(rbB, xvB, ch + 1);
      __builtin_amdgcn_sched_barrier(0);
      TV2_MFMA(rbA, xvA);
      __builtin_amdgcn_sched_barrier(0);
      TV2_LOAD(rbA, xvA, (ch + 2 < cfull ? ch + 2 : ch + 1));
      __builtin_amdgcn_sched_barrier(0);
      TV2_MFMA(rbB, xvB);
      __builtin_amdgcn_sched_barrier(0);
    }
    if (ch < cfull) TV2_MFMA(rbA, xvA);
  } else {
    for (int ch = c0; ch < cfull; ++ch) {
      TV2_LOAD(rbA, xvA, ch);
      TV2_MFMA(rbA, xvA);
    }
  }
  if (c1 > nfull && c0 <= nfull) {
    const int ch = nfull;
    const long k = (long)ch * 16 + 4 * kq;
    const double *rp_ = rp0 + (long)ch * NB * 256;
#pragma unroll
    for (int b = 0; b < NB; ++b) {
      const f64x2 lo = *reinterpret_cast<const f64x2 *>(rp_ + (long)b * 256);
      const f64x2 hi = *reinterpret_cast<const f64x2 *>(rp_ + (long)b * 256 + 2);
      rbA[b][0] = lo.x; rbA[b][1] = lo.y; rbA[b][2] = hi.x; rbA[b][3] = hi.y;
    }
#pragma unroll
    for (int g = 0; g < RG; ++g)
#pragma unroll
      for (int j = 0; j < 4; ++j) xvA[g][j] = (k + j < n) ? xr[g][(long)ch * 16 + j] : 0.0;
    TV2_MFMA(rbA, xvA);
  }
#undef TV2_LOAD
#undef TV2_MFMA
  double *P = a.P + ((long)(kint * a.ksplit + ks) * a.cap) * (NB * 16);
#pragma unroll
  for (int g = 0; g < RG; ++g)
#pragma unroll
    for (int b = 0; b < NB; ++b)
#pragma unroll
      for (int r = 0; r < 4; ++r) {
        const long srow = s0 + g * 16 + kq + 4 * r;
        if (srow < l) P[srow * (NB * 16) + b * 16 + i] = acc[g][b][r];
      }
}
template <bool GATHER>
__global__ __launch_bounds__(256) void table_reduce_kernel(const double *__restrict__ P, int ksplit, long cap, int nb16,
                                                          long l, const int *__restrict__ count, double *__restrict__ T) {
  const int kint = GATHER ? blockIdx.y : 0;
  if (GATHER) l = count[kint];
  const long e = (long)blockIdx.x * 256 + threadIdx.x;
  if (e >= l * nb16) return;
  const long row = e / nb16;
  const int col = (int)(e - row * nb16);
  const double *p = P + ((long)kint * ksplit * cap + row) * nb16 + col;
  double v = 0.0;
  for (int ks = 0; ks < ksplit; ++ks) v += p[(long)ks * cap * nb16];
  if (GATHER)
    T[((long)kint * nb16 + col) * cap + row] = v;
  else
    T[row * nb16 + col] = v;
}
__global__ void grid_weights_multi_kernel(AssocArgs g, GridGeom gg, int c, MultiWeights mw, double *__restrict__ Rp) {
  const int nb = gg.nbx + MULTI_NBA;
  const long total = (long)gg.nc * nb * 256;
  const long e = (long)blockIdx.x * blockDim.x + threadIdx.x;
  if (e >= total) return;
  const int j = (int)(e & 3), col = (int)((e >> 2) & 15), kq = (int)((e >> 6) & 3);
  const long r = e >> 8;
  const int cb = (int)(r % nb);
  const long chunk = r / nb;
  const long k = chunk * 16 + 4 * kq + j;
  double v = 0.0;
  if (k < g.n) {
    if (cb < gg.nbx) {
      const int q = cb * 16 + col;
      if (q < gg.nq) v = grid_weight(g.eval, g.lam_grid, q, k);
    } else {
      const int idx = (cb - gg.nbx) * 16 + col;
      const int a = idx / gg.nq, q = idx - a * gg.nq;
      if (a < c + mw.G) {
        const double u = (a < c) ? g.UtWt[(long)a * g.n + k] : mw.Uty[a - c][k];
        v = u * grid_weight(g.eval, g.lam_grid, q, k);
      }
    }
  }
  Rp[e] = v;
}
__global__ __launch_bounds__(256) void table_multi_reduce_kernel(TableMulti m) {
  const int g = blockIdx.y;
  const long e = (long)blockIdx.x * 256 + threadIdx.x;
  if (e >= m.l * m.nb16) return;
  const long row = e / m.nb16;
  const int col = (int)(e - row * m.nb16);
  int src = col;
  if (col >= m.y0) src = (col - m.y0 < m.nq) ? col + g * m.nq : -1;
  double v = 0.0;
  if (src >= 0) {
    const double *p = m.P + row * m.nb16m + src;
    for (int ks = 0; ks < m.ksplit; ++ks) v += p[(long)ks * m.cap * m.nb16m];
  }
  m.T[(long)g * m.tstride + row * m.nb16 + col] = v;
}

__global__ void cheb_coeff_kernel(const double *__restrict__ eval, int n, ChebNodes nd, const double *__restrict__ Dfit,
                                  int qform, double *__restrict__ Ck, double *__restrict__ Gk, double *__restrict__ Lk,
                                  double *__restrict__ G2k) {
  const int i = blockIdx.x * blockDim.x + threadIdx.x;
  if (i >= n) return;
  const double d = eval[i];
  double hm[CHEB_N], gm[CHEB_N], lm[CHEB_N];
#pragma unroll
  for (int m = 0; m < CHEB_N; ++m) {
    const double ld = nd.lam[m] * d;
    hm[m] = (qform ? d : 1.0) / (ld + 1.0);
    gm[m] = ld / (ld + 1.0);
    lm[m] = log(fabs(ld + 1.0));
  }
  for (int k = 0; k < CHEB_N; ++k) {
    double sh = 0.0, sg = 0.0, sl = 0.0, s2 = 0.0;
#pragma unroll
    for (int m = 0; m < CHEB_N; ++m) {
      const double w = Dfit[k * CHEB_N + m];
      sh += hm[m] * w;
      sg += gm[m] * w;
      sl += lm[m] * w;
      s2 += gm[m] * gm[m] * w;
    }
    Ck[(long)i * CHEB_N + k] = sh;
    Gk[(long)i * CHEB_N + k] = sg;
    Lk[(long)i * CHEB_N + k] = sl;
    G2k[(long)i * CHEB_N + k] = s2;
  }
}

__global__ void cheb_weights_kernel(AssocArgs g, GridGeom gg, int c, const double *__restrict__ Ck,
                                    double *__restrict__ Rp) {
  const long total = (long)gg.nc * (gg.nbx + gg.nba) * 256;
  const long e = (long)blockIdx.x * blockDim.x + threadIdx.x;
  if (e >= total) return;
  const int j = (int)(e & 3), col = (int)((e >> 2) & 15), kq = (int)((e >> 6) & 3);
  const long r = e >> 8;
  const int nb = gg.nbx + gg.nba;
  const int cb = (int)(r % nb);
  const long chunk = r / nb;
  const long k = chunk * 16 + 4 * kq + j;
  double v = 0.0;
  if (k < g.n) {
    if (cb < gg.nbx) {
      const int q = cb * 16 + col;
      if (q < CHEB_N) v = Ck[k * CHEB_N + q];
    } else {
      const int idx = (cb - gg.nbx) * 16 + col;
      const int a = idx / CHEB_N, q = idx - a * CHEB_N;
      if (a <= c) {
        const double u = (a < c) ? g.UtWt[(long)a * g.n + k] : g.Uty[k];
        v = u * Ck[k * CHEB_N + q];
      }
    }
  }
  Rp[e] = v;
}

__global__ __launch_bounds__(256) void cheb_fixed_kernel(AssocArgs g, int c, const double *__restrict__ Ck,
                                                        const double *__restrict__ Gk, const double *__restrict__ Lk,
                                                        const double *__restrict__ G2k, double *__restrict__ F) {
  const int nv = c + 1, npairs = nv * (nv + 1) / 2;
  const int b = blockIdx.x;
  int pa = 0, pb = 0;
  if (b < npairs) {
    int p = 0;
    for (int a = 0; a < nv; ++a)
      for (int bb = a; bb < nv; ++bb, ++p)
        if (p == b) { pa = a; pb = bb; }
  }
  double s[CHEB_N];
#pragma unroll
  for (int k = 0; k < CHEB_N; ++k) s[k] = 0.0;
  for (long i = threadIdx.x; i < g.n; i += 256) {
    double w = 1.0;
    const double *src = (b == npairs) ? Gk : (b == npairs + 1) ? Lk : G2k;
    if (b < npairs) {
      const double ua = (pa < c) ? g.UtWt[(long)pa * g.n + i] : g.Uty[i];
      const double ub = (pb < c) ? g.UtWt[(long)pb * g.n + i] : g.Uty[i];
      w = ua * ub;
      src = Ck;
    }
#pragma unroll
    for (int k = 0; k < CHEB_N; ++k) s[k] += w * src[i * CHEB_N + k];
  }
  __shared__ double red[4][CHEB_N];
  const int lane = threadIdx.x & 63, wave = threadIdx.x >> 6;
#pragma unroll
  for (int k = 0; k < CHEB_N; ++k) {
    const double v = wave_sum(s[k]);
    if (lane == 0) red[wave][k] = v;
  }
  __syncthreads();
  if (threadIdx.x < CHEB_N)
    F[(long)b * CHEB_N + threadIdx.x] =
        ((red[0][threadIdx.x] + red[1][threadIdx.x]) + red[2][threadIdx.x]) + red[3][threadIdx.x];
}
template <int C, bool REML>
__device__ __forceinline__ void cheb_scan_func(const AssocArgs &g, const SnpCtx<FixedC<C>> &cx, const ChebScanArgs &sc,
                                               long snp, int lane) {
  const int func = REML ? 0 : 1;
  double d_lo = dev1_grid<FixedC<C>, REML>(cx, 0);
  for (int i = 0; i < g.n_region; ++i) {
    const double d_hi = dev1_grid<FixedC<C>, REML>(cx, i + 1);
    const int k = i - g.cheb_j0;
    if (d_lo * d_hi <= 0 && k >= 0 && k < g.cheb_nint && lane == 0) {
      int slot = sc.slots[snp * g.cheb_nint + k];
      if (slot < 0) {
        slot = atomicAdd(&sc.count[k], 1);
        sc.list[(long)k * sc.cap + slot] = (int)snp;
        sc.slots[snp * g.cheb_nint + k] = slot;
        sc.dends[((long)(1 - func) * g.cheb_nint + k) * sc.cap + slot] = make_double2(NAN, NAN);
      }
      sc.dends[((long)func * g.cheb_nint + k) * sc.cap + slot] = make_double2(d_lo, d_hi);
    }
    d_lo = d_hi;
  }
}
template <int C>
__global__ __launch_bounds__(256) void cheb_scan_kernel(AssocArgs g, ChebScanArgs sc) {
  const int lane = threadIdx.x & 63;
  const long snp = (long)blockIdx.x * 4 + __builtin_amdgcn_readfirstlane(threadIdx.x >> 6);
  if (snp >= g.l) return;
  SnpCtx<FixedC<C>> cx;
  cx.g = &g;
  cx.x = g.UtX + snp * g.ld;
  cx.y = g.Uty;
  cx.lane = lane;
  cx.m = FixedC<C>();
  cx.logdet_iw = 0.0;
  cx.trow = g.grid_T + snp * g.grid_ld;
  cx.cslots = nullptr;
  if (lane == 0)
    for (int k = 0; k < g.cheb_nint; ++k) sc.slots[snp * g.cheb_nint + k] = -1;
  if (g.a_mode == 1 || g.a_mode == 4) cheb_scan_func<C, true>(g, cx, sc, snp, lane);
  if (g.a_mode == 2 || g.a_mode == 4 || g.a_mode == 9) cheb_scan_func<C, false>(g, cx, sc, snp, lane);
}
template <int C, bool REML>
__device__ __forceinline__ void cheb_search_one(const AssocArgs &g, const ChebSearchArgs &sa, int k, long slot) {
  const int func = REML ? 0 : 1;
  const long e = ((long)func * g.cheb_nint + k) * g.cheb_cap + slot;
  const double2 d = sa.dends[e];
  ChebResult r;
  r.l = 0.0;
  r.status = CHEB_NONE;
  r.pad = 0;
  if (!(d.x != d.x)) {
    ChebEvaluator<C, REML> ev;
    ev.cs.snp = g.cheb_T + (long)k * g.cheb_cap * g.cheb_ld + slot;
    ev.cs.sstride = g.cheb_cap;
    ev.cs.fix = g.cheb_F + (long)k * g.cheb_fld;
    ev.cs.xa0 = g.cheb_xa0;
    ev.cs.mid = sa.mid[k];
    ev.cs.inv_half = sa.inv_half[k];
    ev.cs.n = (double)g.n;
    ev.cs.qform = (int)((sa.qmask >> k) & 1ull);
    ev.cs.s0f = g.grid_F;
#pragma unroll
    for (int a = 0; a < C + 2; ++a) ev.cs.s0x[a] = 0.0;
    if (ev.cs.qform) {
      const double *trow = g.grid_T + (long)sa.list[(long)k * g.cheb_cap + slot] * g.grid_ld;
      ev.cs.s0x[0] = trow[0];
#pragma unroll
      for (int a = 0; a <= C; ++a) ev.cs.s0x[1 + a] = trow[g.grid_xa0 + a * g.grid_nq];
    }
    double l = 0.0, l_temp = 0.0;
    const int j = g.cheb_j0 + k;
    r.status = polish_bracket(ev, g.lam_grid[j], g.lam_grid[j + 1], d.x, d.y, g.l_min, g.l_max, l, l_temp);
    r.l = l;
  }
  sa.res[e] = r;
}
template <int C>
__global__ __launch_bounds__(64) void cheb_search_kernel(AssocArgs g, ChebSearchArgs sa) {
  const int k = blockIdx.y;
  const long slot = (long)blockIdx.x * 64 + threadIdx.x;
  if (slot >= sa.count[k]) return;
  if (blockIdx.z == 0) {
    if (g.a_mode == 1 || g.a_mode == 4) cheb_search_one<C, true>(g, sa, k, slot);
  } else {
    if (g.a_mode == 2 || g.a_mode == 4 || g.a_mode == 9) cheb_search_one<C, false>(g, sa, k, slot);
  }
}

}
```

Before: 364,800.

## Fuse the speculated Chebyshev interval table into the dense table pass

Adds a one-pass mode where the dense grid table kernel also computes the Chebyshev table for a speculated interval (the busiest interval from the previous block), so one read of U^T x serves both tables. Scan and search kernels treat the speculated interval with identity slots instead of atomics and a gather list, and they record the next block's busiest interval. The table kernel's launch grid is also flattened from (rows, ksplit) into per-wave work items, with optional occupancy logging. The cost is more device state, a two-entry ping-pong of the speculated interval, and wasted MFMA work on SNPs whose root lies elsewhere.

Result: no change. 366,000, median of 6 (+0.3%).

```diff
diff --git a/gemma_amd/csrc/abi_lmm_multi.inc.h b/gemma_amd/csrc/abi_lmm_multi.inc.h
--- a/gemma_amd/csrc/abi_lmm_multi.inc.h
+++ b/gemma_amd/csrc/abi_lmm_multi.inc.h
@@ -125,8 +125,7 @@
   a.Rp = g_ctx.multi_R.as<double>() + grp * r_elems;
   a.P = g_ctx.table_P.as<double>(); a.cap = (long)l;
   a.tg = TableGather();
-  const size_t rows_per_block = (size_t)MULTI_RG * 16 * 4;
-  const dim3 grid((unsigned)((l + rows_per_block - 1) / rows_per_block), (unsigned)ksplit);
+  const dim3 grid(table_items(a, l, MULTI_RG * 16, 1));
   if (g_ctx.knobs.table_pf) hipLaunchKernelGGL((table_v2_kernel<2, MULTI_NBA, MULTI_RG, false, true>), grid, dim3(256), 0, s, a);
   else hipLaunchKernelGGL((table_v2_kernel<2, MULTI_NBA, MULTI_RG, false, false>), grid, dim3(256), 0, s, a);
   HIPCHK(hipGetLastError());
diff --git a/gemma_amd/csrc/abi_lmm_stage.inc.h b/gemma_amd/csrc/abi_lmm_stage.inc.h
--- a/gemma_amd/csrc/abi_lmm_stage.inc.h
+++ b/gemma_amd/csrc/abi_lmm_stage.inc.h
@@ -215,6 +215,11 @@
     std::vector<double> ivs(2 * (size_t)nint);
     for (int q = 0; q < nint; ++q) { ivs[2 * q] = p.cheb_mid[q]; ivs[2 * q + 1] = p.cheb_inv_half[q]; }
     HIPCHK(hipMemcpyAsync(g_ctx.cheb_iv.p, ivs.data(), ivs.size() * 8, hipMemcpyHostToDevice, s));
+    if (p.cheb_kstar.reserve(2 * sizeof(int))) return fail(GEMMA_HIP_ENOMEM, "lmm_setup: speculated interval");
+    const int k0 = table_first_interval(a.lam_grid, j0, nint, a.l_mle_null);
+    const int cells[2] = {k0, k0};
+    HIPCHK(hipMemcpyAsync(p.cheb_kstar.p, cells, sizeof cells, hipMemcpyHostToDevice, s));
+    p.cheb_blk = 0;
     HIPCHK(hipStreamSynchronize(s));
   }
   p.cheb_geom = gg;
@@ -267,50 +272,89 @@
 
 static bool table_v2_enabled() { return g_ctx.knobs.table_v2 != 0; }
 static int table_ksplit(int nc) { return std::max(1, std::min(16, nc / 32)); }
+template <typename K>
+static long table_wg_slots(K kernel) {
+  static long slots = 0;
+  if (!slots) {
+    int per_cu = 0;
+    if (hipOccupancyMaxActiveBlocksPerMultiprocessor(&per_cu, kernel, 256, 0) != hipSuccess || per_cu < 1) {
+      (void)hipGetLastError();
+      per_cu = 1;
+    }
+    slots = (long)per_cu * g_ctx.prop.multiProcessorCount;
+  }
+  return slots;
+}
+static unsigned table_items(TableV2 &a, size_t l, int rows, int nsets) {
+  a.nri = table_row_items((long)l, rows);
+  a.nsets = nsets;
+  return (unsigned)table_blocks(a.nri, a.ksplit, nsets);
+}
+template <typename K>
+static void table_note_rounds(const char *what, K kernel, unsigned blocks, unsigned planes) {
+  if (g_ctx.verbose < 2) return;
+  const long slots = table_wg_slots(kernel);
+  const TableRounds r = table_rounds((long)blocks * planes, slots);
+  fprintf(stderr, "[gemma_hip] %s table: %ld workgroups on %ld slots: %ld rounds, %.0f %% filled\n", what, r.blocks, slots, r.rounds,
+          100.0 * r.fill);
+}
+struct TableDual {
+  const double *R2;
+  long r2_stride;
+  const int *kstar;
+  double *T2;
+};
 template <int NBX, int NBA, int RG>
 static int launch_table_v2_t(const GridGeom &gg, const double *UtX, size_t l, size_t ld, const double *R, double *T,
-                             const TableGather *tg, int nint, hipStream_t s) {
+                             const TableGather *tg, int nint, const TableDual *dual, hipStream_t s) {
   constexpr int NB16 = (NBX + NBA) * 16;
-  const size_t rows_per_block = (size_t)RG * 16 * 4;
-  const size_t bx = (l + rows_per_block - 1) / rows_per_block;
   const int ksplit = table_ksplit(gg.nc);
-  const size_t planes = tg ? (size_t)nint : 1;
+  const size_t planes = tg ? (size_t)nint : (dual ? 2 : 1);
   if (g_ctx.table_P.reserve(planes * (size_t)ksplit * l * NB16 * 8))
     return fail(GEMMA_HIP_ENOMEM, "lmm_assoc: table partial sums (%zu bytes)", planes * (size_t)ksplit * l * NB16 * 8);
   TableV2 a;
   a.UtX = UtX; a.ld = (long)ld; a.l = (long)l; a.n = (int)g_ctx.cfg.n; a.nc = gg.nc; a.ksplit = ksplit; a.Rp = R;
   a.P = g_ctx.table_P.as<double>(); a.cap = (long)l;
   if (tg) a.tg = *tg; else a.tg = TableGather();
+  if (dual) { a.Rp2 = dual->R2; a.rp2_stride = dual->r2_stride; a.kstar = dual->kstar; }
   const long total = (long)l * NB16;
   const bool pf = g_ctx.knobs.table_pf != 0;
+  const unsigned bx = table_items(a, l, RG * 16, (!tg && dual) ? 2 : 1);
   if (tg) {
-    if (pf) hipLaunchKernelGGL((table_v2_kernel<NBX, NBA, RG, true, true>), dim3((unsigned)bx, (unsigned)ksplit, (unsigned)nint), dim3(256), 0, s, a);
-    else hipLaunchKernelGGL((table_v2_kernel<NBX, NBA, RG, true, false>), dim3((unsigned)bx, (unsigned)ksplit, (unsigned)nint), dim3(256), 0, s, a);
+    if (pf) hipLaunchKernelGGL((table_v2_kernel<NBX, NBA, RG, true, true>), dim3(bx, (unsigned)nint), dim3(256), 0, s, a);
+    else hipLaunchKernelGGL((table_v2_kernel<NBX, NBA, RG, true, false>), dim3(bx, (unsigned)nint), dim3(256), 0, s, a);
     HIPCHK(hipGetLastError());
     hipLaunchKernelGGL(table_reduce_kernel<true>, dim3((unsigned)((total + 255) / 256), (unsigned)nint), dim3(256), 0, s,
                        a.P, ksplit, a.cap, NB16, (long)l, tg->count, T);
   } else {
-    if (pf) hipLaunchKernelGGL((table_v2_kernel<NBX, NBA, RG, false, true>), dim3((unsigned)bx, (unsigned)ksplit), dim3(256), 0, s, a);
-    else hipLaunchKernelGGL((table_v2_kernel<NBX, NBA, RG, false, false>), dim3((unsigned)bx, (unsigned)ksplit), dim3(256), 0, s, a);
+    if (pf) hipLaunchKernelGGL((table_v2_kernel<NBX, NBA, RG, false, true>), dim3(bx), dim3(256), 0, s, a);
+    else hipLaunchKernelGGL((table_v2_kernel<NBX, NBA, RG, false, false>), dim3(bx), dim3(256), 0, s, a);
     HIPCHK(hipGetLastError());
-    hipLaunchKernelGGL(table_reduce_kernel<false>, dim3((unsigned)((total + 255) / 256)), dim3(256), 0, s, a.P, ksplit,
-                       a.cap, NB16, (long)l, (const int *)nullptr, T);
+    if (pf) table_note_rounds(dual ? "dense + series" : "dense", table_v2_kernel<NBX, NBA, RG, false, true>, bx, 1);
+    else table_note_rounds(dual ? "dense + series" : "dense", table_v2_kernel<NBX, NBA, RG, false, false>, bx, 1);
+    if (dual)
+      hipLaunchKernelGGL(table_reduce_dual_kernel, dim3((unsigned)((total + 255) / 256), 2), dim3(256), 0, s, a.P, ksplit, a.cap,
+                         NB16, (long)l, dual->kstar, T, dual->T2);
+    else
+      hipLaunchKernelGGL(table_reduce_kernel<false>, dim3((unsigned)((total + 255) / 256)), dim3(256), 0, s, a.P, ksplit,
+                         a.cap, NB16, (long)l, (const int *)nullptr, T);
   }
   HIPCHK(hipGetLastError());
   return GEMMA_HIP_OK;
 }
 static int launch_table_v2(const GridGeom &gg, const double *UtX, size_t l, size_t ld, const double *R, double *T,
-                           const TableGather *tg, int nint, hipStream_t s) {
+                           const TableGather *tg, int nint, const TableDual *dual, hipStream_t s) {
   switch (gg.nba) {
-  case 3: return launch_table_v2_t<2, 3, 4>(gg, UtX, l, ld, R, T, tg, nint, s);
-  case 5: return launch_table_v2_t<2, 5, 2>(gg, UtX, l, ld, R, T, tg, nint, s);
-  case 6: return launch_table_v2_t<2, 6, 2>(gg, UtX, l, ld, R, T, tg, nint, s);
-  case 8: return launch_table_v2_t<2, 8, 2>(gg, UtX, l, ld, R, T, tg, nint, s);
+  case 3: return launch_table_v2_t<2, 3, 4>(gg, UtX, l, ld, R, T, tg, nint, dual, s);
+  case 5: return launch_table_v2_t<2, 5, 2>(gg, UtX, l, ld, R, T, tg, nint, dual, s);
+  case 6: return launch_table_v2_t<2, 6, 2>(gg, UtX, l, ld, R, T, tg, nint, dual, s);
+  case 8: return launch_table_v2_t<2, 8, 2>(gg, UtX, l, ld, R, T, tg, nint, dual, s);
   default: return fail(GEMMA_HIP_ERUNTIME, "lmm_assoc: no table kernel for %d column blocks", gg.nba);
   }
 }
 
-static int launch_grid_table(Ctx::PhenoSlot &p, const double *UtX, size_t l, size_t ld, hipStream_t s) {
+static int launch_grid_table(Ctx::PhenoSlot &p, const double *UtX, size_t l, size_t ld, hipStream_t s,
+                             const TableDual *dual = nullptr) {
   const GridGeom &gg = p.grid_geom;
   const size_t nb = (size_t)(gg.nbx + gg.nba);
   if (g_ctx.grid_T.reserve(l * nb * 16 * 8)) return fail(GEMMA_HIP_ENOMEM, "lmm_assoc: fixed-lambda table");
@@ -318,7 +362,7 @@
   const double *R = p.grid_R.as<double>();
   double *T = g_ctx.grid_T.as<double>();
   const int n = (int)g_ctx.cfg.n;
-  if (table_v2_enabled()) return launch_table_v2(gg, UtX, l, ld, R, T, nullptr, 0, s);
+  if (table_v2_enabled()) return launch_table_v2(gg, UtX, l, ld, R, T, nullptr, 0, dual, s);
   switch (gg.nba) {
   case 3: hipLaunchKernelGGL((grid_table_kernel<2, 3, false>), dim3(grid), dim3(256), 0, s, UtX, (long)ld, (long)l, n, gg.nc, R, T, TableGather()); break;
   case 5: hipLaunchKernelGGL((grid_table_kernel<2, 5, false>), dim3(grid), dim3(256), 0, s, UtX, (long)ld, (long)l, n, gg.nc, R, T, TableGather()); break;
@@ -330,14 +374,15 @@
   return GEMMA_HIP_OK;
 }
 
-static int launch_cheb_tables(Ctx::PhenoSlot &p, AssocArgs &a, const double *UtX, size_t l, size_t ld, hipStream_t s) {
+static int launch_cheb_tables(Ctx::PhenoSlot &p, AssocArgs &a, const double *UtX, size_t l, size_t ld, hipStream_t s,
+                              const int *kstar = nullptr, int *kstar_next = nullptr) {
   const GridGeom &gg = p.cheb_geom;
   const size_t nb = (size_t)(gg.nbx + gg.nba), nint = (size_t)a.cheb_nint;
   if (g_ctx.cheb_T.reserve(nint * l * nb * 16 * 8) || g_ctx.cheb_slots.reserve(l * nint * sizeof(int)) ||
-      g_ctx.cheb_list.reserve(nint * l * sizeof(int)) || g_ctx.cheb_count.reserve(ASSOC_MAX_REGION * sizeof(int)) ||
+      g_ctx.cheb_list.reserve(nint * l * sizeof(int)) || g_ctx.cheb_count.reserve((ASSOC_MAX_REGION + 1) * sizeof(int)) ||
       g_ctx.cheb_dends.reserve(2 * nint * l * sizeof(double2)) || g_ctx.cheb_res.reserve(2 * nint * l * sizeof(ChebResult)))
     return fail(GEMMA_HIP_ENOMEM, "lmm_assoc: Chebyshev tables of the batch (%zu bytes)", nint * l * nb * 16 * 8);
-  HIPCHK(hipMemsetAsync(g_ctx.cheb_count.p, 0, ASSOC_MAX_REGION * sizeof(int), s));
+  HIPCHK(hipMemsetAsync(g_ctx.cheb_count.p, 0, (ASSOC_MAX_REGION + 1) * sizeof(int), s));
   a.cheb_T = g_ctx.cheb_T.as<double>();
   a.cheb_cap = (long)l;
   ChebScanArgs sc;
@@ -346,6 +391,8 @@
   sc.slots = g_ctx.cheb_slots.as<int>();
   sc.dends = g_ctx.cheb_dends.as<double2>();
   sc.cap = (long)l;
+  sc.kstar = kstar;
+  sc.nstar = sc.count + ASSOC_MAX_REGION;
   const unsigned sgrid = (unsigned)((l + 3) / 4);
   const size_t c = g_ctx.cfg.n_cvt;
   switch (c) {
@@ -365,7 +412,7 @@
   double *T = g_ctx.cheb_T.as<double>();
   const int n = (int)g_ctx.cfg.n;
   if (table_v2_enabled()) {
-    int rc = launch_table_v2(gg, UtX, l, ld, R, T, &tg, (int)nint, s);
+    int rc = launch_table_v2(gg, UtX, l, ld, R, T, &tg, (int)nint, nullptr, s);
     if (rc) return rc;
   } else
   switch (gg.nba) {
@@ -382,6 +429,9 @@
   sa.qmask = p.cheb_qmask;
   sa.dends = sc.dends;
   sa.res = g_ctx.cheb_res.as<ChebResult>();
+  sa.kstar = kstar;
+  sa.nstar = sc.nstar;
+  sa.kstar_next = kstar_next;
   memcpy(sa.mid, p.cheb_mid, sizeof sa.mid);
   memcpy(sa.inv_half, p.cheb_inv_half, sizeof sa.inv_half);
   const dim3 qgrid((unsigned)((l + 63) / 64), (unsigned)nint, 2);
@@ -491,15 +541,29 @@
     const size_t sel = g_ctx.knobs.force_generic ? 99 : g_ctx.cfg.n_cvt;
     a.grid_T = nullptr;
     if (assoc_takes_tables(a, UtX, ld)) {
-      int rc = shared_T ? GEMMA_HIP_OK : launch_grid_table(p, UtX, l, ld, s);
+      int *kcell = p.cheb_kstar.as<int>();
+      bool onepass = g_ctx.knobs.table_onepass && !shared_T && a.have_cheb && table_v2_enabled() && kcell &&
+                     !g_ctx.cheb_T.reserve((size_t)a.cheb_nint * l * (size_t)a.cheb_ld * 8);
+      TableDual dual;
+      dual.R2 = p.cheb_R.as<double>();
+      dual.r2_stride = (long)p.cheb_geom.nc * (long)(p.cheb_geom.nbx + p.cheb_geom.nba) * 256;
+      dual.kstar = kcell + (p.cheb_blk & 1u);
+      dual.T2 = g_ctx.cheb_T.as<double>();
+      int rc = shared_T ? GEMMA_HIP_OK : launch_grid_table(p, UtX, l, ld, s, onepass ? &dual : nullptr);
+      if (rc == GEMMA_HIP_ENOMEM && onepass) {
+        onepass = false;
+        rc = launch_grid_table(p, UtX, l, ld, s);
+      }
       if (rc && rc != GEMMA_HIP_ENOMEM) return rc;
       a.grid_T = rc ? nullptr : (shared_T ? shared_T : g_ctx.grid_T.as<double>());
       a.cheb_T = nullptr;
       a.cheb_slots = nullptr;
       a.cheb_res = nullptr;
       if (!rc && a.have_cheb) {
-        rc = launch_cheb_tables(p, a, UtX, l, ld, s);
+        rc = onepass ? launch_cheb_tables(p, a, UtX, l, ld, s, dual.kstar, kcell + ((p.cheb_blk + 1) & 1u))
+                     : launch_cheb_tables(p, a, UtX, l, ld, s);
         if (rc && rc != GEMMA_HIP_ENOMEM) return rc;
+        if (!rc && onepass) ++p.cheb_blk;
         if (rc) { a.cheb_T = nullptr; a.cheb_slots = nullptr; a.cheb_res = nullptr; }
       }
     }
diff --git a/gemma_amd/csrc/gemma_hip.hip b/gemma_amd/csrc/gemma_hip.hip
--- a/gemma_amd/csrc/gemma_hip.hip
+++ b/gemma_amd/csrc/gemma_hip.hip
@@ -54,6 +54,7 @@
   int dosage_rows = 16;
   int table_v2 = 1;
   int table_pf = 0;
+  int table_onepass = 1;
   int multi_table = 1;
   int force_generic = 0;
   int assoc_variant = 44;
@@ -102,6 +103,7 @@
     i8.chunks = geti("GEMMA_HIP_OVERLAP_CHUNKS", 4);
     table_v2 = on_unless_0("GEMMA_HIP_TABLE_V2");
     table_pf = off_unless_1("GEMMA_HIP_TABLE_PF");
+    table_onepass = on_unless_0("GEMMA_HIP_TABLE_ONEPASS");
     multi_table = on_unless_0("GEMMA_HIP_MULTI_TABLE");
     force_generic = off_unless_1("GEMMA_HIP_FORCE_GENERIC");
     assoc_variant = geti("GEMMA_HIP_ASSOC_VARIANT", 44);
@@ -206,12 +208,14 @@
     const double *Uty = nullptr;
     DevBuf grid_R, grid_F, cheb_R, cheb_F;
     DevBuf carry;
+    DevBuf cheb_kstar;
+    unsigned cheb_blk = 0;
     GridGeom grid_geom, cheb_geom;
     double cheb_mid[ASSOC_MAX_REGION], cheb_inv_half[ASSOC_MAX_REGION];
     unsigned long long cheb_qmask = 0;
     int carry_flip = 0;
     void release() {
-      grid_R.release(); grid_F.release(); cheb_R.release(); cheb_F.release(); carry.release();
+      grid_R.release(); grid_F.release(); cheb_R.release(); cheb_F.release(); carry.release(); cheb_kstar.release();
       Uty = nullptr;
     }
   };
diff --git a/gemma_amd/csrc/lmm_grid.h b/gemma_amd/csrc/lmm_grid.h
--- a/gemma_amd/csrc/lmm_grid.h
+++ b/gemma_amd/csrc/lmm_grid.h
@@ -2,6 +2,7 @@
 #include <hip/hip_runtime.h>
 #include "dgemm.h"
 #include "lmm_assoc.h"
+#include "table_plan.h"
 
 namespace gemma_hip {
 
@@ -40,6 +41,11 @@
   double *P;
   long cap;
   TableGather tg;
+  long nri = 0;
+  int nsets = 1;
+  const double *Rp2 = nullptr;
+  long rp2_stride = 0;
+  const int *kstar = nullptr;
 };
 
 template <int NBX, int NBA, int RG, bool GATHER, bool PF>
@@ -48,6 +54,10 @@
 template <bool GATHER>
 __global__ __launch_bounds__(256) void table_reduce_kernel(const double *__restrict__ P, int ksplit, long cap, int nb16,
                                                           long l, const int *__restrict__ count, double *__restrict__ T);
+
+__global__ __launch_bounds__(256) void table_reduce_dual_kernel(const double *__restrict__ P, int ksplit, long cap, int nb16,
+                                                               long l, const int *__restrict__ kstar, double *__restrict__ T0,
+                                                               double *__restrict__ T1);
 
 constexpr int MULTI_NBA = 8, MULTI_RG = 2, MULTI_GMAX = 4;
 struct MultiWeights {
@@ -93,6 +103,8 @@
   int *slots;
   double2 *dends;
   long cap;
+  const int *kstar = nullptr;
+  int *nstar = nullptr;
 };
 
 template <int C>
@@ -105,6 +117,8 @@
   const double2 *dends;
   ChebResult *res;
   double mid[ASSOC_MAX_REGION], inv_half[ASSOC_MAX_REGION];
+  const int *kstar = nullptr, *nstar = nullptr;
+  int *kstar_next = nullptr;
 };
 
 template <int C>
diff --git a/gemma_amd/csrc/lmm_grid.hip.h b/gemma_amd/csrc/lmm_grid.hip.h
--- a/gemma_amd/csrc/lmm_grid.hip.h
+++ b/gemma_amd/csrc/lmm_grid.hip.h
@@ -156,16 +156,20 @@
   const int lane = threadIdx.x & 63;
   const int wave = __builtin_amdgcn_readfirstlane(threadIdx.x >> 6);
   const int i = lane & 15, kq = lane >> 4;
-  const int ks = blockIdx.y;
-  const int kint = GATHER ? blockIdx.z : 0;
-  long l = a.l;
+  const int kint = GATHER ? blockIdx.y : 0;
+  long l = a.l, nri = a.nri;
   const double *Rp = a.Rp;
   if (GATHER) {
     l = a.tg.count[kint];
+    nri = table_row_items(l, RG * 16);
     Rp += (long)kint * a.tg.rp_stride;
   }
-  const long s0 = ((long)blockIdx.x * 4 + wave) * (RG * 16);
-  if (s0 >= l) return;
+  const TableItem it = table_item((long)blockIdx.x, wave, nri, a.ksplit, GATHER ? 1 : a.nsets);
+  if (!it.valid) return;
+  const int ks = it.ks;
+  if (!GATHER && it.set) Rp = a.Rp2 + (long)(*a.kstar) * a.rp2_stride;
+  const int plane = GATHER ? kint : it.set;
+  const long s0 = it.ri * (RG * 16);
   const double *xr[RG];
 #pragma unroll
   for (int g = 0; g < RG; ++g) {
@@ -248,7 +252,7 @@
   }
 #undef TV2_LOAD
 #undef TV2_MFMA
-  double *P = a.P + ((long)(kint * a.ksplit + ks) * a.cap) * (NB * 16);
+  double *P = a.P + ((long)(plane * a.ksplit + ks) * a.cap) * (NB * 16);
 #pragma unroll
   for (int g = 0; g < RG; ++g)
 #pragma unroll
@@ -275,6 +279,22 @@
     T[((long)kint * nb16 + col) * cap + row] = v;
   else
     T[row * nb16 + col] = v;
+}
+__global__ __launch_bounds__(256) void table_reduce_dual_kernel(const double *__restrict__ P, int ksplit, long cap, int nb16,
+                                                               long l, const int *__restrict__ kstar, double *__restrict__ T0,
+                                                               double *__restrict__ T1) {
+  const int set = blockIdx.y;
+  const long e = (long)blockIdx.x * 256 + threadIdx.x;
+  if (e >= l * nb16) return;
+  const long row = e / nb16;
+  const int col = (int)(e - row * nb16);
+  const double *p = P + ((long)set * ksplit * cap + row) * nb16 + col;
+  double v = 0.0;
+  for (int ks = 0; ks < ksplit; ++ks) v += p[(long)ks * cap * nb16];
+  if (set)
+    T1[((long)(*kstar) * nb16 + col) * cap + row] = v;
+  else
+    T0[row * nb16 + col] = v;
 }
 __global__ void grid_weights_multi_kernel(AssocArgs g, GridGeom gg, int c, MultiWeights mw, double *__restrict__ Rp) {
   const int nb = gg.nbx + MULTI_NBA;
@@ -418,7 +438,7 @@
 }
 template <int C, bool REML>
 __device__ __forceinline__ void cheb_scan_func(const AssocArgs &g, const SnpCtx<FixedC<C>> &cx, const ChebScanArgs &sc,
-                                               long snp, int lane) {
+                                               long snp, int lane, int kstar) {
   const int func = REML ? 0 : 1;
   double d_lo = dev1_grid<FixedC<C>, REML>(cx, 0);
   for (int i = 0; i < g.n_region; ++i) {
@@ -427,8 +447,13 @@
     if (d_lo * d_hi <= 0 && k >= 0 && k < g.cheb_nint && lane == 0) {
       int slot = sc.slots[snp * g.cheb_nint + k];
       if (slot < 0) {
-        slot = atomicAdd(&sc.count[k], 1);
-        sc.list[(long)k * sc.cap + slot] = (int)snp;
+        if (k == kstar) {
+          slot = (int)snp;
+          atomicAdd(sc.nstar, 1);
+        } else {
+          slot = atomicAdd(&sc.count[k], 1);
+          sc.list[(long)k * sc.cap + slot] = (int)snp;
+        }
         sc.slots[snp * g.cheb_nint + k] = slot;
         sc.dends[((long)(1 - func) * g.cheb_nint + k) * sc.cap + slot] = make_double2(NAN, NAN);
       }
@@ -451,13 +476,19 @@
   cx.logdet_iw = 0.0;
   cx.trow = g.grid_T + snp * g.grid_ld;
   cx.cslots = nullptr;
-  if (lane == 0)
+  const int kstar = sc.kstar ? *sc.kstar : -1;
+  if (lane == 0) {
     for (int k = 0; k < g.cheb_nint; ++k) sc.slots[snp * g.cheb_nint + k] = -1;
-  if (g.a_mode == 1 || g.a_mode == 4) cheb_scan_func<C, true>(g, cx, sc, snp, lane);
-  if (g.a_mode == 2 || g.a_mode == 4 || g.a_mode == 9) cheb_scan_func<C, false>(g, cx, sc, snp, lane);
+    if (kstar >= 0) {
+      sc.dends[((long)kstar) * sc.cap + snp] = make_double2(NAN, NAN);
+      sc.dends[((long)g.cheb_nint + kstar) * sc.cap + snp] = make_double2(NAN, NAN);
+    }
+  }
+  if (g.a_mode == 1 || g.a_mode == 4) cheb_scan_func<C, true>(g, cx, sc, snp, lane, kstar);
+  if (g.a_mode == 2 || g.a_mode == 4 || g.a_mode == 9) cheb_scan_func<C, false>(g, cx, sc, snp, lane, kstar);
 }
 template <int C, bool REML>
-__device__ __forceinline__ void cheb_search_one(const AssocArgs &g, const ChebSearchArgs &sa, int k, long slot) {
+__device__ __forceinline__ void cheb_search_one(const AssocArgs &g, const ChebSearchArgs &sa, int k, long slot, bool star) {
   const int func = REML ? 0 : 1;
   const long e = ((long)func * g.cheb_nint + k) * g.cheb_cap + slot;
   const double2 d = sa.dends[e];
@@ -479,7 +510,7 @@
 #pragma unroll
     for (int a = 0; a < C + 2; ++a) ev.cs.s0x[a] = 0.0;
     if (ev.cs.qform) {
-      const double *trow = g.grid_T + (long)sa.list[(long)k * g.cheb_cap + slot] * g.grid_ld;
+      const double *trow = g.grid_T + (star ? slot : (long)sa.list[(long)k * g.cheb_cap + slot]) * g.grid_ld;
       ev.cs.s0x[0] = trow[0];
 #pragma unroll
       for (int a = 0; a <= C; ++a) ev.cs.s0x[1 + a] = trow[g.grid_xa0 + a * g.grid_nq];
@@ -495,12 +526,23 @@
 __global__ __launch_bounds__(64) void cheb_search_kernel(AssocArgs g, ChebSearchArgs sa) {
   const int k = blockIdx.y;
   const long slot = (long)blockIdx.x * 64 + threadIdx.x;
-  if (slot >= sa.count[k]) return;
+  const int kstar = sa.kstar ? *sa.kstar : -1;
+  if (sa.kstar_next && blockIdx.x == 0 && blockIdx.y == 0 && blockIdx.z == 0 && threadIdx.x == 0) {
+    int best = kstar >= 0 ? kstar : 0;
+    int nbest = kstar >= 0 ? *sa.nstar : sa.count[0];
+    for (int q = 0; q < g.cheb_nint; ++q) {
+      const int nq = (q == kstar) ? *sa.nstar : sa.count[q];
+      if (nq > nbest) { best = q; nbest = nq; }
+    }
+    *sa.kstar_next = best;
+  }
+  const bool star = (k == kstar);
+  if (slot >= (star ? g.l : (long)sa.count[k])) return;
   if (blockIdx.z == 0) {
-    if (g.a_mode == 1 || g.a_mode == 4) cheb_search_one<C, true>(g, sa, k, slot);
+    if (g.a_mode == 1 || g.a_mode == 4) cheb_search_one<C, true>(g, sa, k, slot, star);
   } else {
-    if (g.a_mode == 2 || g.a_mode == 4 || g.a_mode == 9) cheb_search_one<C, false>(g, sa, k, slot);
-  }
-}
-
-}
+    if (g.a_mode == 2 || g.a_mode == 4 || g.a_mode == 9) cheb_search_one<C, false>(g, sa, k, slot, star);
+  }
+}
+
+}
diff --git a/gemma_amd/csrc/table_plan.h b/gemma_amd/csrc/table_plan.h
--- /dev/null
+++ b/gemma_amd/csrc/table_plan.h
@@ -0,0 +1,56 @@
+#pragma once
+
+#if defined(__HIPCC__)
+#define TABLE_PLAN_FN __host__ __device__ inline
+#else
+#define TABLE_PLAN_FN inline
+#endif
+
+namespace gemma_hip {
+
+constexpr int TABLE_WG_WAVES = 4;
+
+struct TableItem {
+  long ri;
+  int ks;
+  int set;
+  bool valid;
+};
+
+TABLE_PLAN_FN long table_row_items(long l, int rows) { return (l + rows - 1) / rows; }
+TABLE_PLAN_FN long table_pairs(long nri, int ksplit) { return nri * (long)ksplit; }
+TABLE_PLAN_FN long table_blocks(long nri, int ksplit, int nsets) {
+  const long per = TABLE_WG_WAVES / nsets;
+  return (table_pairs(nri, ksplit) + per - 1) / per;
+}
+TABLE_PLAN_FN TableItem table_item(long block, int wave, long nri, int ksplit, int nsets) {
+  const int per = TABLE_WG_WAVES / nsets;
+  TableItem it;
+  it.set = wave / per;
+  const long q = block * per + (wave - it.set * per);
+  it.valid = nri > 0 && q < table_pairs(nri, ksplit);
+  it.ks = it.valid ? (int)(q / nri) : 0;
+  it.ri = it.valid ? q - (long)it.ks * nri : 0;
+  return it;
+}
+
+struct TableRounds {
+  long blocks, rounds;
+  double fill;
+};
+inline TableRounds table_rounds(long blocks, long wg_slots) {
+  TableRounds r;
+  r.blocks = blocks;
+  r.rounds = wg_slots > 0 ? (blocks + wg_slots - 1) / wg_slots : 0;
+  r.fill = r.rounds > 0 ? (double)blocks / ((double)r.rounds * (double)wg_slots) : 0.0;
+  return r;
+}
+
+inline int table_first_interval(const double *lam_grid, int j0, int nint, double l_null) {
+  int k = 0;
+  if (l_null == l_null)
+    while (k + 1 < nint && l_null >= lam_grid[j0 + k + 1]) ++k;
+  return k;
+}
+
+}
```
